# DanielLin94144/E2E-ASR-Pytorch

Measured on NVIDIA B200. Metric: beam-8+LM joint CTC/attn decode utts/sec, higher is better.
Workload: dtype f32

## Files before the change

e2e-asr-pytorch_b200/_lib.py:

```python
import ctypes
import os

from . import build as _build

c_int, c_float, c_void_p = ctypes.c_int, ctypes.c_float, ctypes.c_void_p

CTC_LOGZERO = -100000000.0
DEC_LOG_ZERO = -10000000.0
STATUS_PREFIX_TOO_LONG = 1
STATUS_TOKEN_NOT_CAND = 2
PREFIX_FULL = 1
PREFIX_SKIP_DEAD_ROWS = 2
PREFIX_FAST_MATH = 4
PREFIX_LIBM_MATH = 8
PREFIX_ROW_COPIES = 16
PREFIX_POLY_MATH = 32
PREFIX_POLY_ESTRIN = 64
BEAM_USE_CTC = 1
BEAM_USE_LM = 2

SIGNATURES = {
    "e2e_last_error": (ctypes.c_char_p, []),
    "e2e_abi_version": (c_int, []),
    "e2e_padded_vocab": (c_int, [c_int]),
    "e2e_launch_count": (ctypes.c_longlong, []),
    "e2e_add_launch_count": (None, [ctypes.c_longlong]),
    "e2e_ctc_log_softmax": (c_int, [c_void_p, c_int, c_int, c_int, c_void_p, c_int, c_void_p, c_int, c_void_p]),
    "e2e_ctc_init_state": (c_int, [c_void_p, c_int, c_int, c_int, c_void_p, c_void_p, c_void_p]),
    "e2e_ctc_prefix_score": (c_int, [c_void_p, c_int, c_int, c_int, c_int, c_void_p,
                                     c_void_p, c_int,
                                     c_void_p, c_void_p, c_void_p,
                                     c_void_p, c_void_p, c_int, c_int, c_int,
                                     c_void_p, c_void_p, c_void_p, c_int, c_void_p]),
    "e2e_ctc_prefix_step_supported": (c_int, [c_int, c_int, c_int]),
    "e2e_ctc_prefix_step": (c_int, [c_void_p, c_int, c_int, c_int, c_int, c_void_p,
                                    c_void_p, c_int,
                                    c_void_p, c_void_p, c_void_p, c_void_p,
                                    c_void_p, c_void_p, c_int, c_int, c_int,
                                    c_void_p, c_void_p, c_void_p, c_int, c_void_p]),
    "e2e_beam_candidates": (c_int, [c_void_p, c_int, c_int, c_int, c_int, c_int, c_void_p, c_void_p, c_void_p, c_void_p]),
    "e2e_beam_combine_prune": (c_int, [c_void_p, c_int, c_void_p,
                                       c_void_p, c_int,
                                       c_void_p, c_void_p,
                                       c_int, c_int, c_int, c_int, c_int,
                                       c_void_p, c_void_p,
                                       c_float, c_float, c_float, c_int,
                                       c_void_p, c_void_p, c_void_p, c_void_p,
                                       c_void_p, c_void_p, c_void_p,
                                       c_void_p,
                                       c_void_p, c_void_p, c_void_p,
                                       c_void_p, c_void_p, c_void_p, c_void_p, c_void_p,
                                       c_int, c_void_p, c_int, c_void_p, c_void_p, c_void_p, c_void_p]),
    "e2e_attention_loc_full": (c_int, [c_void_p, c_void_p, c_void_p, c_void_p, c_void_p, c_void_p, c_void_p, c_void_p,
                                       c_float, c_float, c_int, c_int, c_int, c_int, c_int, c_int, c_int, c_int,
                                       c_void_p, c_void_p, c_void_p]),
    "e2e_attention_loc_heads_supported": (c_int, [c_int, c_int, c_int, c_int, c_int]),
    "e2e_attention_loc_heads": (c_int, [c_void_p, c_void_p, c_void_p, c_void_p, c_void_p, c_void_p, c_void_p, c_void_p,
                                        c_float, c_float, c_int, c_int, c_int, c_int, c_int, c_int, c_int, c_int,
                                        c_int, c_int, c_void_p, c_void_p, c_void_p]),
    "e2e_lstm_split_rows": (c_int, [c_void_p, ctypes.c_longlong, c_void_p, c_int, c_int, c_void_p, ctypes.c_longlong, c_int, c_int, c_void_p]),
    "e2e_lstm_split_rows_multi": (c_int, [c_int, c_void_p, c_void_p, c_void_p, c_void_p, c_void_p, c_void_p, c_void_p, c_void_p, c_int, c_void_p]),
    "e2e_lstm_cell": (c_int, [c_void_p, ctypes.c_longlong, c_void_p, c_void_p, c_void_p, c_void_p, c_void_p, c_int, c_int,
                              c_void_p, c_void_p, c_void_p, ctypes.c_longlong, c_int, c_int, c_void_p]),
    "e2e_lstm_split_rows_f16x2": (c_int, [c_void_p, ctypes.c_longlong, c_void_p, c_int, c_int, c_void_p, ctypes.c_longlong, c_int, c_int,
                                          c_float, c_void_p]),
    "e2e_lstm_split_rows_multi_f16x2": (c_int, [c_int, c_void_p, c_void_p, c_void_p, c_void_p, c_void_p, c_void_p, c_void_p, c_void_p,
                                                c_int, c_float, c_void_p]),
    "e2e_lstm_cell_f16x2": (c_int, [c_void_p, ctypes.c_longlong, c_float, c_void_p, c_void_p, c_void_p, c_void_p, c_void_p, c_int, c_int,
                                    c_void_p, c_void_p, c_void_p, ctypes.c_longlong, c_int, c_int, c_float, c_void_p]),
    "e2e_gru_cell": (c_int, [c_void_p, ctypes.c_longlong, c_void_p, c_void_p, c_void_p, c_void_p, c_void_p, c_int, c_int,
                             c_void_p, c_void_p, ctypes.c_longlong, c_int, c_int, c_void_p]),
    "e2e_gru_cell_f16x2": (c_int, [c_void_p, ctypes.c_longlong, c_float, c_void_p, c_void_p, c_void_p, c_void_p, c_void_p, c_int, c_int,
                                   c_void_p, c_void_p, ctypes.c_longlong, c_int, c_int, c_float, c_void_p]),
    "e2e_conv3x3_unfold_split": (c_int, [c_void_p, c_void_p, c_int, c_int, c_int, c_int, ctypes.c_longlong, c_int, c_void_p, c_void_p]),
    "e2e_conv_bias_relu_mask": (c_int, [c_void_p, c_void_p, c_void_p, c_int, c_int, c_int, c_int, ctypes.c_longlong,
                                        ctypes.c_longlong, c_void_p]),
    "e2e_conv3x3_igemm_supported": (c_int, [c_int, c_int]),
    "e2e_conv3x3_igemm": (c_int, [c_void_p, c_void_p, c_int, c_int, c_int, c_int, c_void_p, c_void_p, c_int, c_int, c_void_p, c_void_p]),
    "e2e_lstm_sequence": (c_int, [c_void_p, ctypes.c_longlong, c_void_p, ctypes.c_longlong, c_void_p, c_void_p, c_void_p, c_void_p,
                                  c_int, c_int, c_int, c_int,
                                  c_void_p, c_void_p, c_int, c_int, c_void_p, c_void_p, c_int, c_int, c_void_p]),
    "e2e_gru_sequence": (c_int, [c_void_p, ctypes.c_longlong, c_void_p, ctypes.c_longlong, c_void_p, c_void_p, c_void_p, c_void_p,
                                 c_int, c_int, c_int, c_int,
                                 c_void_p, c_void_p, c_int, c_int, c_void_p, c_void_p, c_int, c_int, c_void_p]),
    "e2e_conv1_direct": (c_int, [c_void_p, ctypes.c_longlong, c_void_p, c_void_p, c_void_p, c_int, c_int, c_int, c_int, c_int,
                                 c_void_p, c_void_p]),
    "e2e_conv_bias_relu_mask_pool": (c_int, [c_void_p, c_void_p, c_void_p, c_int, c_int, c_int, c_int, c_void_p, c_void_p]),
    "e2e_conv1_direct_amax": (c_int, [c_void_p, ctypes.c_longlong, c_void_p, c_void_p, c_void_p, c_int, c_int, c_int, c_int, c_int,
                                      c_void_p, c_void_p, c_void_p]),
    "e2e_conv3x3_unfold_split_f16x2": (c_int, [c_void_p, c_void_p, c_int, c_int, c_int, c_int, ctypes.c_longlong, c_int, c_void_p,
                                               c_void_p, c_void_p]),
    "e2e_conv_bias_relu_mask_scaled": (c_int, [c_void_p, c_void_p, c_void_p, c_int, c_int, c_int, c_int, ctypes.c_longlong,
                                               ctypes.c_longlong, c_void_p, c_float, c_void_p, c_void_p]),
    "e2e_conv_bias_relu_mask_pool_scaled": (c_int, [c_void_p, c_void_p, c_void_p, c_int, c_int, c_int, c_int, c_void_p, c_void_p, c_float,
                                                    c_void_p, c_void_p]),
    "e2e_nbest_pack_ragged": (c_int, [c_int, c_int, c_int, c_void_p, c_void_p, c_void_p, c_void_p, c_void_p, c_void_p, c_void_p,
                                      c_void_p, c_void_p, c_void_p, c_void_p, c_void_p]),
    "e2e_copy_rows_h2d": (c_int, [c_void_p, c_void_p, ctypes.c_longlong, c_int, c_void_p, c_void_p, c_int, c_int, c_void_p, c_void_p]),
    "e2e_beam_finalize": (c_int, [c_int, c_int, c_void_p,
                                  c_void_p, c_void_p,
                                  c_void_p, c_void_p, c_void_p,
                                  c_void_p, c_void_p, c_void_p,
                                  c_void_p, c_void_p, c_int,
                                  c_void_p, c_void_p, c_void_p, c_void_p, c_void_p,
                                  c_int, c_void_p]),
}

_lib = None


class E2EError(RuntimeError):
    pass


def load():
    global _lib
    if _lib is None:
        path = os.environ.get("E2E_ASR_B200_LIB")
        if not path:
            path = _build.LIB_PATH
            if _build.stale():
                path = _build.build()
        lib = ctypes.CDLL(path)
        for name, (res, args) in SIGNATURES.items():
            fn = getattr(lib, name)
            fn.restype, fn.argtypes = res, args
        if lib.e2e_abi_version() != 1:
            raise E2EError("libe2e_asr_b200.so ABI version mismatch")
        _lib = lib
    return _lib


def check(rc):
    if rc != 0:
        raise E2EError("libe2e_asr_b200: rc=%d: %s" % (rc, load().e2e_last_error().decode()))


def ptr(t):
    return None if t is None else t.data_ptr()


def require_cuda(*tensors):
    for t in tensors:
        if t is not None and not t.is_cuda:
            raise E2EError("libe2e_asr_b200 has no CPU path: tensor on %s" % t.device)
```

e2e-asr-pytorch_b200/csrc/conv_igemm.cu:

```cuda
#include "common.cuh"
#include "conv_igemm.cuh"
#include <cuda_bf16.h>

namespace e2e {
namespace {

constexpr int kBM = kIgemmBM, kBN = kIgemmBN, kBK = kIgemmBK;
constexpr int kTile = kBM * kBK * 2;
constexpr int kBStages = 6;
constexpr int kBarBytes = 256;
constexpr int kGroups = 3;
constexpr int kAStages = 2 * kGroups;
constexpr int kThreads = 64 + 128 * kGroups;
constexpr int kSmemBytes = 1024 + (kAStages + kBStages) * kTile + kBarBytes + kBM * 16;

static_assert((2 * (kAStages + kBStages) + 1) * 8 + 4 <= kBarBytes, "barrier block");

constexpr uint32_t kIdesc = (1u << 4) | (1u << 7) | (1u << 10) | ((uint32_t)(kBN >> 3) << 17) | ((uint32_t)(kBM >> 4) << 24);

__device__ __forceinline__ uint64_t sw128_desc(uint32_t saddr)
{
    return (uint64_t)((saddr >> 4) & 0x3fffu) | ((uint64_t)1 << 16) | ((uint64_t)(1024 >> 4) << 32) | ((uint64_t)1 << 46) |
           ((uint64_t)2 << 61);
}

__device__ __forceinline__ void mbar_arrive(uint64_t *bar)
{
    asm volatile("mbarrier.arrive.shared::cta.b64 _, [%0];" ::"r"(smem_u32(bar)) : "memory");
}

__device__ __forceinline__ void tma_load_2d(void *dst, const CUtensorMap *map, int c0, int c1, uint64_t *bar)
{
    asm volatile("cp.async.bulk.tensor.2d.shared::cluster.global.tile.mbarrier::complete_tx::bytes [%0], [%1, {%2, %3}], [%4];"
                 ::"r"(smem_u32(dst)), "l"(map), "r"(c0), "r"(c1), "r"(smem_u32(bar))
                 : "memory");
}

__device__ __forceinline__ void tc_fence_after() { asm volatile("tcgen05.fence::after_thread_sync;" ::: "memory"); }
__device__ __forceinline__ void tc_fence_before() { asm volatile("tcgen05.fence::before_thread_sync;" ::: "memory"); }

__device__ __forceinline__ void tc_mma(uint32_t d_tmem, uint64_t adesc, uint64_t bdesc, uint32_t accumulate)
{
    asm volatile("{\n\t.reg .pred p;\n\tsetp.ne.b32 p, %4, 0;\n\t"
                 "tcgen05.mma.cta_group::1.kind::f16 [%0], %1, %2, %3, p;\n\t}"
                 ::"r"(d_tmem), "l"(adesc), "l"(bdesc), "r"(kIdesc), "r"(accumulate));
}

__device__ __forceinline__ void tc_commit(uint64_t *bar)
{
    asm volatile("tcgen05.commit.cta_group::1.mbarrier::arrive::one.shared::cluster.b64 [%0];" ::"r"(smem_u32(bar)) : "memory");
}

__device__ __forceinline__ void tmem_ld32(uint32_t taddr, float (&v)[32])
{
    uint32_t *r = reinterpret_cast<uint32_t *>(v);
    asm volatile("tcgen05.ld.sync.aligned.32x32b.x32.b32 {%0, %1, %2, %3, %4, %5, %6, %7, %8, %9, %10, %11, %12, %13, %14, %15, "
                 "%16, %17, %18, %19, %20, %21, %22, %23, %24, %25, %26, %27, %28, %29, %30, %31}, [%32];"
                 : "=r"(r[0]), "=r"(r[1]), "=r"(r[2]), "=r"(r[3]), "=r"(r[4]), "=r"(r[5]), "=r"(r[6]), "=r"(r[7]),
                   "=r"(r[8]), "=r"(r[9]), "=r"(r[10]), "=r"(r[11]), "=r"(r[12]), "=r"(r[13]), "=r"(r[14]), "=r"(r[15]),
                   "=r"(r[16]), "=r"(r[17]), "=r"(r[18]), "=r"(r[19]), "=r"(r[20]), "=r"(r[21]), "=r"(r[22]), "=r"(r[23]),
                   "=r"(r[24]), "=r"(r[25]), "=r"(r[26]), "=r"(r[27]), "=r"(r[28]), "=r"(r[29]), "=r"(r[30]), "=r"(r[31])
                 : "r"(taddr));
}

__device__ __forceinline__ uint32_t split_piece2(float x0, float x1, int pp)
{
    __nv_bfloat162 p = __floats2bfloat162_rn(x0, x1);
    if (pp > 0) {
        const float2 a = __bfloat1622float2(p);
        x0 = __fsub_rn(x0, a.x);
        x1 = __fsub_rn(x1, a.y);
        p = __floats2bfloat162_rn(x0, x1);
        if (pp > 1) {
            const float2 b = __bfloat1622float2(p);
            p = __floats2bfloat162_rn(__fsub_rn(x0, b.x), __fsub_rn(x1, b.y));
        }
    }
    return *reinterpret_cast<uint32_t *>(&p);
}

struct alignas(16) IgemmRow {
    const float *pix;
    uint32_t flags;
    uint32_t pad;
};
constexpr uint32_t kRowLive = 1u << 9, kRowPixel = 1u << 10;

__global__ void __launch_bounds__(kThreads, 1)
conv3x3_igemm_kernel(const __grid_constant__ CUtensorMap wmap, const IgemmArgs args)
{
    extern __shared__ uint8_t igemm_smem_raw[];
    uint8_t *smem = reinterpret_cast<uint8_t *>((reinterpret_cast<uintptr_t>(igemm_smem_raw) + 1023) & ~(uintptr_t)1023);
    uint8_t *a_ring = smem;
    uint8_t *b_ring = smem + kAStages * kTile;
    uint64_t *bars = reinterpret_cast<uint64_t *>(b_ring + kBStages * kTile);
    uint64_t *a_full = bars, *a_empty = bars + kAStages;
    uint64_t *b_full = bars + 2 * kAStages, *b_empty = b_full + kBStages;
    uint64_t *acc_full = b_empty + kBStages;
    uint32_t *tmem_slot = reinterpret_cast<uint32_t *>(acc_full + 1);
    IgemmRow *rows = reinterpret_cast<IgemmRow *>(reinterpret_cast<uint8_t *>(bars) + kBarBytes);

    const int warp = threadIdx.x >> 5, lane = threadIdx.x & 31;
    const int H = args.H, W = args.W, C = args.C;
    const bool pool = args.epi == kEpiPool;
    const int n0 = blockIdx.y * kBN;
    const int KB = 9 * C / kBK;

    if (threadIdx.x == 0) {
        for (int i = 0; i < kAStages; ++i) { mbar_init(a_full + i, 128); mbar_init(a_empty + i, 1); }
        for (int i = 0; i < kBStages; ++i) { mbar_init(b_full + i, 1); mbar_init(b_empty + i, 1); }
        mbar_init(acc_full, 1);
        mbar_fence_init();
    }
    if (warp == 0) {
        asm volatile("tcgen05.alloc.cta_group::1.sync.aligned.shared::cta.b32 [%0], 512;" ::"r"(smem_u32(tmem_slot)) : "memory");
        asm volatile("tcgen05.relinquish_alloc_permit.cta_group::1.sync.aligned;" ::: "memory");
    }
    if (threadIdx.x >= 64 && threadIdx.x < 64 + kBM) {
        const int m = threadIdx.x - 64;
        int h = 0, w = 0, n = -1;
        if (pool) {
            const int H2 = (H + 1) >> 1, W2 = (W + 1) >> 1;
            const long long q = (long long)blockIdx.x * (kBM / 4) + (m >> 2);
            if (q < (long long)args.N * H2 * W2) {
                const int w2 = (int)(q % W2);
                const long long t = q / W2;
                h = 2 * (int)(t % H2) + ((m >> 1) & 1);
                w = 2 * w2 + (m & 1);
                if (h < H && w < W) n = (int)(t / H2);
            }
        } else {
            const long long p = (long long)blockIdx.x * kBM + m;
            if (p < (long long)args.N * H * W) {
                const long long t = p / W;
                w = (int)(p % W);
                h = (int)(t % H);
                n = (int)(t / H);
            }
        }
        IgemmRow r = {args.in, 0u, 0u};
        if (n >= 0) {
            const int vr = __ldg(args.valid + n);
            r.pix = args.in + (((long long)n * H + h) * W + w) * C;
            r.flags = kRowPixel | (h < vr ? kRowLive : 0u);
            for (int t = 0; t < 9; ++t) {
                const int hs = h + t / 3 - 1, ws = w + t % 3 - 1;
                if (hs >= 0 && hs < H && hs < vr && ws >= 0 && ws < W) r.flags |= 1u << t;
            }
        }
        rows[m] = r;
    }
    tc_fence_before();
    __syncthreads();
    tc_fence_after();
    const uint32_t tmem = *tmem_slot;

    if (warp == 0) {
        if (lane == 0) {
            int stage = 0;
            uint32_t phase = 0;
            for (int pp = 0; pp < 3; ++pp)
                for (int kb = 0; kb < KB; ++kb)
                    for (int j = 0; j < 3 - pp; ++j) {
                        mbar_wait(b_empty + stage, phase ^ 1u);
                        mbar_arrive_expect_tx(b_full + stage, kTile);
                        tma_load_2d(b_ring + stage * kTile, &wmap, kb * kBK, j * args.Cout + n0, b_full + stage);
                        if (++stage == kBStages) { stage = 0; phase ^= 1u; }
                    }
        }
    } else if (warp == 1) {
        if (lane == 0) {
            int as = 0, bs = 0;
            uint32_t aph = 0, bph = 0;
            for (int pp = 0; pp < 3; ++pp)
                for (int kb = 0; kb < KB; ++kb) {
                    mbar_wait(a_full + as, aph);
                    tc_fence_after();
                    const uint64_t adesc = sw128_desc(smem_u32(a_ring + as * kTile));
                    for (int j = 0; j < 3 - pp; ++j) {
                        mbar_wait(b_full + bs, bph);
                        tc_fence_after();
                        const uint64_t bdesc = sw128_desc(smem_u32(b_ring + bs * kTile));
#pragma unroll
                        for (int k16 = 0; k16 < kBK / 16; ++k16)
                            tc_mma(tmem + (uint32_t)((pp + j) * kBN), adesc + 2 * k16, bdesc + 2 * k16,
                                   (pp > 0 || kb > 0 || k16 > 0) ? 1u : 0u);
                        tc_commit(b_empty + bs);
                        if (++bs == kBStages) { bs = 0; bph ^= 1u; }
                    }
                    tc_commit(a_empty + as);
                    if (++as == kAStages) { as = 0; aph ^= 1u; }
                }
            tc_commit(acc_full);
        }
    } else {
        const int grp = (threadIdx.x - 64) >> 7, pt = (threadIdx.x - 64) & 127;
        const int c16 = pt & 15, rsub = pt >> 4;
        const int cpb = C / kBK;
        int as = grp;
        uint32_t aph = 0;
        for (int seq = grp; seq < 3 * KB; seq += kGroups) {
            const int pp = seq / KB, kb = seq - pp * KB, tap = kb / cpb, cb = kb - tap * cpb;
            const long long tap_off = ((long long)(tap / 3 - 1) * W + (tap % 3 - 1)) * C + cb * kBK + c16 * 4;
            float4 v[kBM / 8];
#pragma unroll
            for (int i = 0; i < kBM / 8; ++i) {
                const IgemmRow r = rows[i * 8 + rsub];
                v[i] = make_float4(0.0f, 0.0f, 0.0f, 0.0f);
                if ((r.flags >> tap) & 1u) v[i] = __ldg(reinterpret_cast<const float4 *>(r.pix + tap_off));
            }
            mbar_wait(a_empty + as, aph ^ 1u);
            uint8_t *tile = a_ring + as * kTile;
#pragma unroll
            for (int i = 0; i < kBM / 8; ++i) {
                const int row = i * 8 + rsub;
                const uint32_t lo = split_piece2(v[i].x, v[i].y, pp), hi = split_piece2(v[i].z, v[i].w, pp);
                const int chunk = (c16 >> 1) ^ (row & 7);
                *reinterpret_cast<uint2 *>(tile + row * 128 + chunk * 16 + (c16 & 1) * 8) = make_uint2(lo, hi);
            }
            asm volatile("fence.proxy.async.shared::cta;" ::: "memory");
            mbar_arrive(a_full + as);
            as += kGroups;
            if (as >= kAStages) { as -= kAStages; aph ^= 1u; }
        }

        const int m = (warp & 3) * 32 + lane;
        const uint32_t flags = rows[m].flags;
        mbar_wait(acc_full, 0);
        tc_fence_after();
        const uint32_t lane_addr = tmem + ((uint32_t)((warp & 3) * 32) << 16);
        const long long H2W2 = (long long)((H + 1) >> 1) * ((W + 1) >> 1);
        const bool live = (flags & kRowLive) != 0u, pixel = (flags & kRowPixel) != 0u;
        for (int c = grp; c < kBN / 32; c += kGroups) {
            float y0[32], y1[32], y2[32];
            tmem_ld32(lane_addr + c * 32, y0);
            tmem_ld32(lane_addr + kBN + c * 32, y1);
            tmem_ld32(lane_addr + 2 * kBN + c * 32, y2);
            asm volatile("tcgen05.wait::ld.sync.aligned;" ::: "memory");
            float y[32];
#pragma unroll
            for (int i = 0; i < 32; ++i) y[i] = __fadd_rn(y0[i], __fadd_rn(y1[i], y2[i]));
            const int col = n0 + c * 32;
            if (args.epi == kEpiRaw) {
                if (pixel) {
                    float4 *dst = reinterpret_cast<float4 *>(args.out + ((long long)blockIdx.x * kBM + m) * args.Cout + col);
#pragma unroll
                    for (int i = 0; i < 8; ++i) dst[i] = make_float4(y[4 * i], y[4 * i + 1], y[4 * i + 2], y[4 * i + 3]);
                }
            } else if (!pool) {
                if (pixel) {
                    float4 *dst = reinterpret_cast<float4 *>(args.out + ((long long)blockIdx.x * kBM + m) * args.Cout + col);
#pragma unroll
                    for (int i = 0; i < 8; ++i) {
                        float4 o = make_float4(0.0f, 0.0f, 0.0f, 0.0f);
                        if (live) {
                            const float4 b = __ldg(reinterpret_cast<const float4 *>(args.bias + col) + i);
                            o.x = fmaxf(__fadd_rn(y[4 * i], b.x), 0.0f); o.y = fmaxf(__fadd_rn(y[4 * i + 1], b.y), 0.0f);
                            o.z = fmaxf(__fadd_rn(y[4 * i + 2], b.z), 0.0f); o.w = fmaxf(__fadd_rn(y[4 * i + 3], b.w), 0.0f);
                        }
                        dst[i] = o;
                    }
                }
            } else {
                const int s = m & 3, base = lane & ~3;
                float t[32];
#pragma unroll
                for (int i = 0; i < 32; ++i) t[i] = live ? __fadd_rn(y[i], __ldg(args.bias + col + i)) : -INFINITY;
                float res[8];
#pragma unroll
                for (int i = 0; i < 32; ++i) {
                    float acc = 0.0f;
#pragma unroll
                    for (int k = 0; k < 4; ++k) acc = fmaxf(acc, __shfl_sync(E2E_FULL_MASK, t[i], base + k));
                    if ((i >> 3) == s) res[i & 7] = acc;
                }
                const long long q = (long long)blockIdx.x * (kBM / 4) + (m >> 2);
                if (q < (long long)args.N * H2W2) {
                    float4 *dst = reinterpret_cast<float4 *>(args.out + q * args.Cout + col + 8 * s);
                    dst[0] = make_float4(res[0], res[1], res[2], res[3]);
                    dst[1] = make_float4(res[4], res[5], res[6], res[7]);
                }
            }
        }
        tc_fence_before();
    }
    __syncthreads();
    if (warp == 0) asm volatile("tcgen05.dealloc.cta_group::1.sync.aligned.b32 %0, 512;" ::"r"(tmem) : "memory");
}

}
}

extern "C" int e2e_tc_conv3x3_igemm_launch(const CUtensorMap *wmap, const e2e::IgemmArgs *args, unsigned tiles, void *stream)
{
    using namespace e2e;
    static bool attr_set = false;
    if (!attr_set) {
        const cudaError_t e = cudaFuncSetAttribute(conv3x3_igemm_kernel, cudaFuncAttributeMaxDynamicSharedMemorySize, kSmemBytes);
        if (e != cudaSuccess) return (int)e;
        attr_set = true;
    }
    conv3x3_igemm_kernel<<<dim3(tiles, (unsigned)(args->Cout / kBN)), kThreads, kSmemBytes, static_cast<cudaStream_t>(stream)>>>(*wmap, *args);
    return (int)cudaGetLastError();
}
```

e2e-asr-pytorch_b200/csrc/conv_igemm.cuh:

```cuda
#pragma once
#include <cuda.h>
#include <cuda_runtime.h>

namespace e2e {

constexpr int kIgemmBM = 128;
constexpr int kIgemmBN = 128;
constexpr int kIgemmBK = 64;

enum { kEpiRaw = 0, kEpiRelu = 1, kEpiPool = 2 };

struct IgemmArgs {
    const float *in;
    const int *valid;
    const float *bias;
    float *out;
    int N, H, W, C, Cout, epi;
};

}

extern "C" int e2e_tc_conv3x3_igemm_launch(const CUtensorMap *wmap, const e2e::IgemmArgs *args, unsigned tiles, void *stream);
```

e2e-asr-pytorch_b200/csrc/conv_igemm_host.cu:

```cuda
#include "common.cuh"
#include "conv_igemm.cuh"

namespace e2e {

typedef CUresult (*EncodeTiledFn)(CUtensorMap *, CUtensorMapDataType, cuuint32_t, void *, const cuuint64_t *, const cuuint64_t *,
                                  const cuuint32_t *, const cuuint32_t *, CUtensorMapInterleave, CUtensorMapSwizzle,
                                  CUtensorMapL2promotion, CUtensorMapFloatOOBfill);
EncodeTiledFn tensor_map_encoder();

namespace {

bool igemm_shape_ok(int C, int Cout)
{
    return (C == 128 || C == 256) && (Cout == 128 || Cout == 256);
}

}
}

using namespace e2e;

extern "C" int e2e_conv3x3_igemm_supported(int C, int Cout)
{
    return igemm_shape_ok(C, Cout) ? 1 : 0;
}

extern "C" int e2e_conv3x3_igemm(const float *in_nhwc, const int *valid_rows, int N, int H, int W, int C,
                                 const void *w_split_bf16, const float *bias, int Cout, int epilogue, float *out, void *stream)
{
    const char *name = "e2e_conv3x3_igemm";
    if (!in_nhwc || !valid_rows || !w_split_bf16 || !out || (epilogue != kEpiRaw && !bias))
        return set_error(E2E_ERR_ARG, "%s: null pointer", name);
    if (N <= 0 || H <= 0 || W <= 0 || epilogue < kEpiRaw || epilogue > kEpiPool)
        return set_error(E2E_ERR_ARG, "%s: bad size or epilogue", name);
    if (!igemm_shape_ok(C, Cout)) return set_error(E2E_ERR_UNSUPPORTED, "%s: C = %d, Cout = %d not supported", name, C, Cout);
    if ((reinterpret_cast<uintptr_t>(in_nhwc) & 15) || (reinterpret_cast<uintptr_t>(w_split_bf16) & 15) ||
        (reinterpret_cast<uintptr_t>(out) & 15) || (reinterpret_cast<uintptr_t>(bias) & 15))
        return set_error(E2E_ERR_ARG, "%s: misaligned buffer", name);
    const long long rows_out = epilogue == kEpiPool ? (long long)N * ((H + 1) / 2) * ((W + 1) / 2) : (long long)N * H * W;
    const long long tiles = epilogue == kEpiPool ? (rows_out + kIgemmBM / 4 - 1) / (kIgemmBM / 4) : (rows_out + kIgemmBM - 1) / kIgemmBM;
    if (tiles > 0x7fffffffLL) return set_error(E2E_ERR_ARG, "%s: too many pixels", name);

    EncodeTiledFn enc = tensor_map_encoder();
    if (!enc) return set_error(E2E_ERR_LAUNCH, "%s: cuTensorMapEncodeTiled is not available from this driver", name);
    CUtensorMap map;
    const cuuint64_t dims[2] = {(cuuint64_t)9 * C, (cuuint64_t)3 * Cout};
    const cuuint64_t strides[1] = {(cuuint64_t)9 * C * 2};
    const cuuint32_t box[2] = {(cuuint32_t)kIgemmBK, (cuuint32_t)kIgemmBN};
    const cuuint32_t estr[2] = {1u, 1u};
    const CUresult cr = enc(&map, CU_TENSOR_MAP_DATA_TYPE_BFLOAT16, 2, const_cast<void *>(w_split_bf16), dims, strides, box, estr,
                            CU_TENSOR_MAP_INTERLEAVE_NONE, CU_TENSOR_MAP_SWIZZLE_128B, CU_TENSOR_MAP_L2_PROMOTION_L2_256B,
                            CU_TENSOR_MAP_FLOAT_OOB_FILL_NONE);
    if (cr != CUDA_SUCCESS) return set_error(E2E_ERR_LAUNCH, "%s: cuTensorMapEncodeTiled failed (CUresult %d)", name, (int)cr);

    const IgemmArgs a = {in_nhwc, valid_rows, bias, out, N, H, W, C, Cout, epilogue};
    const int e = e2e_tc_conv3x3_igemm_launch(&map, &a, (unsigned)tiles, stream);
    count_launch();
    if (e != (int)cudaSuccess) return set_error(E2E_ERR_LAUNCH, "%s: %s", name, cudaGetErrorString((cudaError_t)e));
    return check_launch(name);
}
```

e2e-asr-pytorch_b200/model.py:

```python
import math

import numpy as np
import torch
from torch import nn
import torch.nn.functional as F

FBANK_SIZE = 40


def reference_init_(module):
    if isinstance(module, nn.Embedding):
        module.weight.data.normal_(0, 1)
        return
    for p in module.parameters():
        d = p.data
        if d.dim() == 1:
            d.zero_()
        elif d.dim() == 2:
            d.normal_(0, 1.0 / math.sqrt(d.size(1)))
        elif d.dim() in (3, 4):
            fan = d.size(1)
            for k in d.size()[2:]:
                fan *= k
            d.normal_(0, 1.0 / math.sqrt(fan))
        else:
            raise NotImplementedError


def split_gemm_rows(x, lin, a_bytes=3 << 30):
    from . import ops
    f, k = x.shape
    m_out = lin.b0.shape[1]
    y = torch.empty((f, m_out), dtype=torch.float32, device=x.device)
    blk = max(1, min(f, a_bytes // (3 * k * 2)))
    a = torch.empty((blk, 3 * k), dtype=torch.bfloat16, device=x.device)
    for r0 in range(0, f, blk):
        m = min(blk, f - r0)
        ops.lstm_split_rows(x[r0:r0 + m], None, m, a, k, 0)
        am, ym = a[:m], y[r0:r0 + m]
        torch.mm(am, lin.b2, out_dtype=torch.float32, out=ym)
        torch.addmm(ym, am[:, :2 * k], lin.b1, out_dtype=torch.float32, out=ym)
        torch.addmm(ym, am[:, :k], lin.b0, out_dtype=torch.float32, out=ym)
    return y


class VGGFrontEnd(nn.Module):

    def __init__(self, input_dim):
        super().__init__()
        if input_dim % 13 == 0:
            self.in_channel, self.freq_dim = input_dim // 13, 13
        elif input_dim % FBANK_SIZE == 0:
            self.in_channel, self.freq_dim = input_dim // FBANK_SIZE, FBANK_SIZE
        else:
            raise ValueError("VGG front end needs 13k (MFCC) or 40k (fbank) features, got %d" % input_dim)
        c1, c2 = 128, 256
        self.out_dim = (self.freq_dim // 4) * c2
        self.extractor = nn.Sequential(
            nn.Conv2d(self.in_channel, c1, 3, stride=1, padding=1), nn.ReLU(),
            nn.Conv2d(c1, c1, 3, stride=1, padding=1), nn.ReLU(),
            nn.MaxPool2d(2, stride=2, ceil_mode=True),
            nn.Conv2d(c1, c2, 3, stride=1, padding=1), nn.ReLU(),
            nn.Conv2d(c2, c2, 3, stride=1, padding=1), nn.ReLU(),
            nn.MaxPool2d(2, stride=2, ceil_mode=True))

    def _as_image(self, feat):
        drop = feat.shape[1] % 4
        if drop:
            feat = feat[:, :-drop, :].contiguous()
        n, t, _ = feat.shape
        return feat.view(n, t, self.in_channel, self.freq_dim).transpose(1, 2)

    def forward(self, feat, feat_len):
        img = self.extractor(self._as_image(feat))
        out = img.transpose(1, 2).contiguous()
        return out.view(out.shape[0], out.shape[1], self.out_dim), feat_len // 4

    def forward_masked(self, feat, feat_len):
        img = self._as_image(feat)
        n, _, t, _ = img.shape
        own = (feat_len // 4 * 4).to(img.device)

        def keep(a):
            valid = own // (t // a.shape[2])
            m = torch.arange(a.shape[2], device=a.device)[None, :] < valid[:, None]
            return a * m[:, None, :, None].to(a.dtype)

        img = keep(img)
        for layer in self.extractor:
            img = layer(img)
            if isinstance(layer, nn.ReLU):
                img = keep(img)
        out = img.transpose(1, 2).contiguous()
        return out.view(out.shape[0], out.shape[1], self.out_dim), feat_len // 4


    A_BYTES = 3 << 30

    conv_split_format = "bf16x3"
    conv_path = "igemm"
    IGEMM_MAX_COUT = 128

    def _split_weights(self, conv):
        from .stepper import SplitLinear, SplitLinearF16
        cache = self.__dict__.setdefault("_split_cache", {})
        key = (id(conv), conv.weight.device, self.conv_split_format)
        if key not in cache:
            w2d = conv.weight.detach().permute(2, 3, 1, 0).reshape(-1, conv.out_channels).t().contiguous()
            cache[key] = SplitLinearF16(w2d, act_scale=1.0) if self.conv_split_format == "fp16x2" else SplitLinear(w2d)
        return cache[key]

    def _igemm_weights(self, conv):
        cache = self.__dict__.setdefault("_split_cache", {})
        key = (id(conv), conv.weight.device, "igemm")
        if key not in cache:
            lin, k = self._split_weights(conv), 9 * conv.in_channels
            cache[key] = torch.stack([lin.b0.t(), lin.b1[:k].t(), lin.b2[:k].t()]).contiguous()
        return cache[key]

    def _conv_split(self, x, valid, conv, pool=False, amax_in=None, amax_out=None):
        from . import ops
        n, h, w, c = x.shape
        bias = conv.bias.detach().float().contiguous()
        if (amax_in is None and self.conv_path == "igemm" and conv.out_channels <= self.IGEMM_MAX_COUT
                and ops.conv3x3_igemm_supported(c, conv.out_channels)):
            return ops.conv3x3_igemm(x, valid, self._igemm_weights(conv), bias, "pool" if pool else "relu")
        k = 9 * c
        lin = self._split_weights(conv)
        total = n * h * w
        f16 = amax_in is not None
        pieces, a_dtype = (2, torch.float16) if f16 else (3, torch.bfloat16)
        blk = max(1, min(total, self.A_BYTES // (pieces * k * 2)))
        a = torch.empty((blk, pieces * k), dtype=a_dtype, device=x.device)
        y = torch.empty((total, conv.out_channels), dtype=torch.float32, device=x.device)
        for p0 in range(0, total, blk):
            m = min(blk, total - p0)
            ops.conv3x3_unfold_split(x, valid, p0, m, a, amax=amax_in)
            am, ym = a[:m], y[p0:p0 + m]
            if f16:
                torch.mm(am, lin.b1, out_dtype=torch.float32, out=ym)
            else:
                torch.mm(am, lin.b2, out_dtype=torch.float32, out=ym)
                torch.addmm(ym, am[:, :2 * k], lin.b1, out_dtype=torch.float32, out=ym)
            torch.addmm(ym, am[:, :k], lin.b0, out_dtype=torch.float32, out=ym)
        y = y.view(n, h, w, conv.out_channels)
        scale_args = (amax_in, lin.out_scale, amax_out) if f16 else ()
        if pool:
            return ops.conv_bias_relu_mask_pool(y, bias, valid, *scale_args)
        ops.conv_bias_relu_mask(y, bias, valid, *scale_args)
        return y

    def forward_masked_split(self, feat, feat_len):
        from . import ops
        drop = feat.shape[1] % 4
        if drop:
            feat = feat[:, :-drop, :]
        if feat.stride(2) != 1 or feat.stride(1) != feat.shape[2]:
            feat = feat.contiguous()
        own = (feat_len // 4 * 4).to(feat.device)
        v1 = own.to(torch.int32).contiguous()
        v2 = (own // 2).to(torch.int32).contiguous()
        convs = [m for m in self.extractor if isinstance(m, nn.Conv2d)]
        w1 = convs[0].weight.detach().float().contiguous()
        f16 = self.conv_split_format == "fp16x2"
        amax = torch.zeros(4, dtype=torch.int32, device=feat.device) if f16 else None
        word = lambda i: amax[i:i + 1] if f16 else None
        y = ops.conv1_direct(feat, w1, convs[0].bias.detach().float().contiguous(), v1, self.freq_dim, amax_out=word(0))
        y = self._conv_split(y, v1, convs[1], pool=True, amax_in=word(0), amax_out=word(1))
        y = self._conv_split(y, v2, convs[2], amax_in=word(1), amax_out=word(2))
        y = self._conv_split(y, v2, convs[3], pool=True, amax_in=word(2), amax_out=word(3))
        out = y.permute(0, 1, 3, 2).contiguous()
        return out.view(out.shape[0], out.shape[1], self.out_dim), feat_len // 4


class RecurrentLayer(nn.Module):

    def __init__(self, input_dim, module, dim, bidirection, dropout, layer_norm, sample_rate, sample_style, proj):
        super().__init__()
        if sample_style not in ("drop", "concat"):
            raise ValueError("Unsupported Sample Style: " + sample_style)
        width = 2 * dim if bidirection else dim
        self.out_dim = sample_rate * width if (sample_rate > 1 and sample_style == "concat") else width
        self.sample_rate, self.sample_style = sample_rate, sample_style
        self.dropout, self.layer_norm, self.proj = dropout, layer_norm, proj
        self.layer = getattr(nn, module.upper())(input_dim, dim, bidirectional=bidirection, num_layers=1, batch_first=True)
        if layer_norm:
            self.ln = nn.LayerNorm(width)
        if dropout > 0:
            self.dp = nn.Dropout(p=dropout)
        if proj:
            self.pj = nn.Linear(width, width)

    def _post(self, out, x_len):
        if self.layer_norm:
            out = self.ln(out)
        if self.dropout > 0:
            out = self.dp(out)
        if self.sample_rate > 1:
            n, t, d = out.shape
            x_len = x_len // self.sample_rate
            if self.sample_style == "drop":
                out = out[:, ::self.sample_rate, :].contiguous()
            else:
                if t % self.sample_rate:
                    out = out[:, :-(t % self.sample_rate), :]
                out = out.contiguous().view(n, t // self.sample_rate, d * self.sample_rate)
        if self.proj:
            out = torch.tanh(self.pj(out))
        return out, x_len

    def forward(self, x, x_len):
        out, _ = self.layer(x)
        return self._post(out, x_len)

    def forward_ragged(self, x, x_len):
        rnn = self.layer
        if not rnn.bidirectional:
            out, _ = rnn(x)
            return self._post(out, x_len)
        n, t, _ = x.shape
        fn = torch._VF.lstm if isinstance(rnn, nn.LSTM) else torch._VF.gru
        zeros = x.new_zeros(1, n, rnn.hidden_size)
        hx = (zeros, zeros) if isinstance(rnn, nn.LSTM) else zeros
        names = ("weight_ih_l0", "weight_hh_l0", "bias_ih_l0", "bias_hh_l0")
        w_fw = [getattr(rnn, k) for k in names]
        w_bw = [getattr(rnn, k + "_reverse") for k in names]
        ar = torch.arange(t, device=x.device)[None, :]
        ln = x_len.to(x.device).clamp(min=1)[:, None]
        rev = torch.where(ar < ln, ln - 1 - ar, ar)
        gather = rev[:, :, None]
        fw = fn(x, hx, w_fw, True, 1, 0.0, False, False, True)[0]
        x_rev = x.gather(1, gather.expand(n, t, x.shape[2]))
        bw = fn(x_rev, hx, w_bw, True, 1, 0.0, False, False, True)[0]
        bw = bw.gather(1, gather.expand(n, t, bw.shape[2]))
        return self._post(torch.cat([fw, bw], dim=-1), x_len)


    def packed_supported(self):
        rnn = self.layer
        return (isinstance(rnn, (nn.LSTM, nn.GRU)) and rnn.num_layers == 1 and self.sample_rate == 1 and not self.layer_norm
                and rnn.hidden_size <= 384)

    def _packed_weights(self):
        from .stepper import SplitLinear
        rnn = self.layer
        cache = self.__dict__.setdefault("_packed_cache", {})
        key = rnn.weight_hh_l0.device
        if key not in cache:
            sfx = ["", "_reverse"] if rnn.bidirectional else [""]
            g = lambda n: getattr(rnn, n).detach().float()
            h = rnn.hidden_size
            w_in = torch.cat([g("weight_ih_l0" + x) for x in sfx], dim=0)
            if isinstance(rnn, nn.LSTM):
                dirs = [((g("bias_ih_l0" + x) + g("bias_hh_l0" + x)).contiguous(),
                         g("weight_hh_l0" + x).view(4, h, h).permute(2, 1, 0).contiguous())
                        for x in sfx]
            else:
                dirs = []
                for x in sfx:
                    b_ih, b_hh, w_hh = g("bias_ih_l0" + x), g("bias_hh_l0" + x), g("weight_hh_l0" + x).view(3, h, h)
                    bias = torch.cat([b_ih[:2 * h] + b_hh[:2 * h], b_ih[2 * h:], b_hh[2 * h:]]).contiguous()
                    w_t = torch.cat([w_hh, w_hh.new_zeros(1, h, h)]).permute(2, 1, 0).contiguous()
                    dirs.append((bias, w_t))
            pj = (SplitLinear(self.pj.weight.detach().float()), self.pj.bias.detach().float()) if self.proj else None
            cache[key] = (SplitLinear(w_in), dirs, pj)
        return cache[key]

    def forward_packed(self, x, frame_off, lens32, group_first, group_rows):
        from . import ops
        lin_in, dirs, pj = self._packed_weights()
        h = self.layer.hidden_size
        gru = isinstance(self.layer, nn.GRU)
        n_gates = 3 if gru else 4
        gates = split_gemm_rows(x.contiguous(), lin_in)
        out = torch.empty((x.shape[0], h * len(dirs)), dtype=torch.float32, device=x.device)
        fw = (dirs[0][0], dirs[0][1], 0, 0)
        bw = (dirs[1][0], dirs[1][1], n_gates * h, h) if len(dirs) == 2 else None
        (ops.gru_sequence if gru else ops.lstm_sequence)(gates, out, frame_off, lens32, group_first, group_rows, h, fw, bw)
        if pj is not None:
            out = torch.tanh(split_gemm_rows(out, pj[0]).add_(pj[1]))
        return out


class Encoder(nn.Module):

    def __init__(self, input_size, batch_size, vgg, vgg_freq, vgg_low_filt, module, bidirection, dim, dropout,
                 layer_norm, proj, sample_rate, sample_style):
        super().__init__()
        assert len(sample_rate) == len(dropout) == len(dim), "Number of layer mismatch"
        self.vgg, self.vgg_freq, self.vgg_low_filt = vgg, vgg_freq, vgg_low_filt
        self.sample_rate = 1
        stack, width = [], input_size
        if vgg == 1:
            stack.append(VGGFrontEnd(input_size))
            width = stack[-1].out_dim
            self.sample_rate *= 4
        elif vgg != 0:
            raise NotImplementedError("vgg = {} front end is outside the decode hot path scope".format(vgg))
        if module not in ("LSTM", "GRU"):
            raise NotImplementedError("encoder module " + str(module))
        for l in range(len(dim)):
            stack.append(RecurrentLayer(width, module, dim[l], bidirection, dropout[l], layer_norm[l],
                                        sample_rate[l], sample_style, proj[l]))
            width = stack[-1].out_dim
            self.sample_rate *= sample_rate[l]
        self.in_dim, self.out_dim = input_size, width
        self.layers = nn.ModuleList(stack)

    def forward(self, x, x_len):
        for layer in self.layers:
            x, x_len = layer(x, x_len)
        return x, x_len

    def packed_supported(self):
        return all(isinstance(l, VGGFrontEnd) or (isinstance(l, RecurrentLayer) and l.packed_supported()) for l in self.layers)

    @staticmethod
    def _groups(t_host):
        first, rows, i, n = [], [], 0, len(t_host)
        while i < n:
            t = int(t_host[i])
            r = 4 if t >= 600 else (8 if t >= 300 else 16)
            r = min(r, n - i)
            first.append(i)
            rows.append(r)
            i += r
        return first, rows

    def forward_ragged_packed(self, x, x_len, chunk=128):
        lens_host = x_len.cpu()
        n_utts = x.shape[0]
        front = self.layers[0] if isinstance(self.layers[0], VGGFrontEnd) else None
        packs, tls = [], []
        ready = getattr(self, "chunk_ready", None)
        for lo in range(0, n_utts, chunk):
            hi = min(n_utts, lo + chunk)
            if ready is not None:
                ready(lo, hi)
            l_max = int(lens_host[lo:hi].max())
            xc, lc = x[lo:hi, :l_max], x_len[lo:hi]
            if front is not None:
                if getattr(self, "split_conv", False):
                    xc, lc = front.forward_masked_split(xc, lc)
                else:
                    xc, lc = front.forward_masked(xc, lc)
            lc = lc.to(x.device).reshape(-1)
            mask = torch.arange(xc.shape[1], device=x.device)[None, :] < lc[:, None]
            packs.append(xc[mask])
            tls.append(lc)
        feat = torch.cat(packs, dim=0)
        t_len = torch.cat(tls).long()
        t_host = t_len.cpu()
        frame_off = (torch.cumsum(t_len, 0) - t_len).to(torch.int32).contiguous()
        lens32 = t_len.to(torch.int32).contiguous()
        first, rows = self._groups(t_host)
        g_first = torch.tensor(first, dtype=torch.int32, device=x.device)
        g_rows = torch.tensor(rows, dtype=torch.int32, device=x.device)
        for layer in self.layers:
            if isinstance(layer, RecurrentLayer):
                feat = layer.forward_packed(feat, frame_off, lens32, g_first, g_rows)
        t_max = int(t_host.max())
        enc = feat.new_zeros((n_utts, t_max, feat.shape[1]))
        enc[torch.arange(t_max, device=x.device)[None, :] < t_len[:, None]] = feat
        return enc, t_len

    def forward_ragged(self, x, x_len):
        for layer in self.layers:
            if isinstance(layer, VGGFrontEnd):
                if getattr(self, "split_conv", False) and x.is_cuda:
                    x, x_len = layer.forward_masked_split(x, x_len)
                else:
                    x, x_len = layer.forward_masked(x, x_len)
            else:
                x, x_len = layer.forward_ragged(x, x_len)
        return x, x_len


class _AttentionCore(nn.Module):

    def __init__(self, temperature, num_head):
        super().__init__()
        self.temperature, self.num_head = temperature, num_head
        self.mask, self.k_len = None, None

    def reset_mem(self):
        self.mask, self.k_len = None, None

    def set_mem(self, prev_att):
        pass

    def compute_mask(self, k, k_len):
        self.k_len = k_len
        n, t, _ = k.shape
        pad = torch.arange(t, device=k_len.device)[None, :] >= k_len[:, None]
        self.mask = pad[:, None, :].expand(n, self.num_head, t).reshape(-1, t)

    def _attend(self, energy, value):
        score = (energy / self.temperature).masked_fill(self.mask, -np.inf)
        attn = torch.softmax(score, dim=-1)
        return torch.bmm(attn.unsqueeze(1), value).squeeze(1), attn


class ScaleDotAttention(_AttentionCore):
    def forward(self, q, k, v):
        energy = torch.bmm(q.unsqueeze(1), k.transpose(1, 2)).squeeze(1)
        out, attn = self._attend(energy, v)
        return out, attn.view(-1, self.num_head, k.shape[1])


class LocationAwareAttention(_AttentionCore):

    def __init__(self, kernel_size, kernel_num, dim, num_head, temperature):
        super().__init__(temperature, num_head)
        self.prev_att = None
        self.loc_conv = nn.Conv1d(num_head, kernel_num, kernel_size=2 * kernel_size + 1, padding=kernel_size, bias=False)
        self.loc_proj = nn.Linear(kernel_num, dim, bias=False)
        self.gen_energy = nn.Linear(dim, 1)
        self.dim = dim

    def reset_mem(self):
        super().reset_mem()
        self.prev_att = None

    def set_mem(self, prev_att):
        self.prev_att = prev_att

    def forward(self, q, k, v):
        nh, t, _ = k.shape
        n = nh // self.num_head
        if self.prev_att is None:
            self.prev_att = torch.zeros((n, self.num_head, t), device=k.device)
            for i, sl in enumerate(self.k_len):
                self.prev_att[i, :, :sl] = 1.0 / sl
        loc = torch.tanh(self.loc_proj(self.loc_conv(self.prev_att).transpose(1, 2)))
        loc = loc.unsqueeze(1).repeat(1, self.num_head, 1, 1).view(-1, t, self.dim)
        energy = self.gen_energy(torch.tanh(k + q.unsqueeze(1) + loc)).squeeze(2)
        out, attn = self._attend(energy, v)
        attn = attn.view(n, self.num_head, t)
        self.prev_att = attn
        return out, attn


class Attention(nn.Module):

    def __init__(self, v_dim, q_dim, mode, dim, num_head, temperature, v_proj, loc_kernel_size, loc_kernel_num):
        super().__init__()
        self.v_dim, self.dim, self.mode, self.num_head, self.v_proj = v_dim, dim, mode.lower(), num_head, v_proj
        self.proj_q = nn.Linear(q_dim, dim * num_head)
        self.proj_k = nn.Linear(v_dim, dim * num_head)
        if v_proj:
            self.proj_v = nn.Linear(v_dim, v_dim * num_head)
        if self.mode == "dot":
            self.att_layer = ScaleDotAttention(temperature, num_head)
        elif self.mode == "loc":
            self.att_layer = LocationAwareAttention(loc_kernel_size, loc_kernel_num, dim, num_head, temperature)
        else:
            raise NotImplementedError
        if num_head > 1:
            self.merge_head = nn.Linear(v_dim * num_head, v_dim)
        self.key = self.value = self.mask = None

    def reset_mem(self):
        self.key = self.value = self.mask = None
        self.att_layer.reset_mem()

    def set_mem(self, prev_attn):
        self.att_layer.set_mem(prev_attn)

    def forward(self, dec_state, enc_feat, enc_len):
        n, t, _ = enc_feat.shape
        query = torch.tanh(self.proj_q(dec_state)).view(n * self.num_head, self.dim)
        if self.key is None:
            self.att_layer.compute_mask(enc_feat, enc_len.to(enc_feat.device))
            self.key = torch.tanh(self.proj_k(enc_feat))
            self.value = torch.tanh(self.proj_v(enc_feat)) if self.v_proj else enc_feat
            if self.num_head > 1:
                self.key = self.key.view(n, t, self.num_head, self.dim).permute(0, 2, 1, 3).contiguous().view(-1, t, self.dim)
                if self.v_proj:
                    self.value = self.value.view(n, t, self.num_head, self.v_dim).permute(0, 2, 1, 3).contiguous().view(-1, t, self.v_dim)
                else:
                    self.value = self.value.repeat(self.num_head, 1, 1)
        context, attn = self.att_layer(query, self.key, self.value)
        if self.num_head > 1:
            context = self.merge_head(context.view(n, self.num_head * self.v_dim))
        return attn, context


class Decoder(nn.Module):

    def __init__(self, batch_size, input_dim, vocab_size, module, dim, layer, dropout):
        super().__init__()
        if module not in ("LSTM", "GRU"):
            raise NotImplementedError("decoder module " + str(module))
        self.in_dim, self.layer, self.dim, self.dropout = input_dim, layer, dim, dropout
        self.hidden_state = None
        self.enable_cell = module == "LSTM"
        self.layers = getattr(nn, module)(input_dim, dim, num_layers=layer, dropout=dropout, batch_first=True)
        self.char_trans = nn.Linear(dim, vocab_size)
        self.final_dropout = nn.Dropout(dropout)

    def init_state(self, bs):
        dev = next(self.parameters()).device
        z = lambda: torch.zeros((self.layer, bs, self.dim), device=dev)
        self.hidden_state = (z(), z()) if self.enable_cell else z()
        return self.get_state()

    def set_state(self, hidden_state):
        dev = next(self.parameters()).device
        if self.enable_cell:
            self.hidden_state = (hidden_state[0].to(dev), hidden_state[1].to(dev))
        else:
            self.hidden_state = hidden_state.to(dev)

    def get_state(self):
        if self.enable_cell:
            return (self.hidden_state[0].cpu(), self.hidden_state[1].cpu())
        return self.hidden_state.cpu()

    def get_query(self):
        h = self.hidden_state[0] if self.enable_cell else self.hidden_state
        return h.transpose(0, 1).reshape(-1, self.dim * self.layer)

    def forward(self, x):
        x, self.hidden_state = self.layers(x.unsqueeze(1), self.hidden_state)
        x = x.squeeze(1)
        return self.char_trans(self.final_dropout(x)), x


class ASR(nn.Module):

    def __init__(self, input_size, vocab_size, batch_size, ctc_weight, encoder, attention, decoder,
                 emb_drop=0.0, init_adadelta=True):
        super().__init__()
        assert 0 <= ctc_weight <= 1
        self.vocab_size, self.ctc_weight = vocab_size, ctc_weight
        self.enable_ctc, self.enable_att = ctc_weight > 0, ctc_weight != 1
        self.lm = None
        self.encoder = Encoder(input_size, batch_size, **encoder)
        if self.enable_ctc:
            self.ctc_layer = nn.Sequential(nn.Linear(self.encoder.out_dim, vocab_size), nn.ReLU())
        if self.enable_att:
            self.dec_dim = decoder["dim"]
            self.pre_embed = nn.Embedding(vocab_size, self.dec_dim)
            self.embed_drop = nn.Dropout(emb_drop)
            self.decoder = Decoder(batch_size, self.encoder.out_dim + self.dec_dim, vocab_size, **decoder)
            self.attention = Attention(self.encoder.out_dim, self.dec_dim * self.decoder.layer, **attention)
        self.apply(reference_init_)
        if self.enable_att and self.decoder.enable_cell:
            for l in range(self.decoder.layer):
                b = getattr(self.decoder.layers, "bias_ih_l{}".format(l))
                n = b.size(0)
                b.data[n // 4:n // 2].fill_(1.0)

    def set_state(self, prev_state, prev_attn):
        self.decoder.set_state(prev_state)
        self.attention.set_mem(prev_attn)

    def forward(self, *a, **k):
        raise NotImplementedError("training forward (asr.py:89-177) is outside the decode hot-path scope")


class RNNLM(nn.Module):

    def __init__(self, vocab_size, emb_tying, emb_dim, module, dim, n_layers, dropout):
        super().__init__()
        self.dim, self.n_layers, self.emb_tying, self.vocab_size = dim, n_layers, emb_tying, vocab_size
        if emb_tying:
            assert emb_dim == dim, "Output dim of RNN should be identical to embedding if using weight tying."
        self.emb = nn.Embedding(vocab_size, emb_dim)
        self.dp1, self.dp2 = nn.Dropout(dropout), nn.Dropout(dropout)
        self.rnn = getattr(nn, module.upper())(emb_dim, dim, num_layers=n_layers, dropout=dropout, batch_first=True)
        if not emb_tying:
            self.trans = nn.Linear(emb_dim, vocab_size)

    def forward(self, x, lens, hidden=None):
        emb = self.dp1(self.emb(x))
        packed = nn.utils.rnn.pack_padded_sequence(emb, lens, batch_first=True, enforce_sorted=False)
        out, hidden = self.rnn(packed, hidden)
        out, _ = nn.utils.rnn.pad_packed_sequence(out, batch_first=True)
        out = F.linear(self.dp2(out), self.emb.weight) if self.emb_tying else self.trans(self.dp2(out))
        return out, hidden
```

e2e-asr-pytorch_b200/ops.py:

```python
import torch

from . import _lib as L

I32, F32 = torch.int32, torch.float32


def _stream():
    return torch.cuda.current_stream().cuda_stream


def _chk(t, dtype, name, numel=None):
    if t is None:
        return
    if not t.is_cuda:
        raise L.E2EError("%s must be a CUDA tensor (no CPU path)" % name)
    if t.dtype != dtype:
        raise TypeError("%s must be %s, got %s" % (name, dtype, t.dtype))
    if not t.is_contiguous():
        raise ValueError("%s must be contiguous" % name)
    if numel is not None and t.numel() < numel:
        raise ValueError("%s has %d elements, needs %d" % (name, t.numel(), numel))


def padded_vocab(v):
    return L.load().e2e_padded_vocab(int(v))


def ctc_log_softmax(logits, enc_len=None, apply_relu=True, out=None):
    _chk(logits, F32, "logits")
    _chk(enc_len, I32, "enc_len")
    u, t, v = logits.shape
    vp = padded_vocab(v)
    x = out if out is not None else torch.empty((t, u, vp), dtype=F32, device=logits.device)
    _chk(x, F32, "x", t * u * vp)
    L.check(L.load().e2e_ctc_log_softmax(L.ptr(logits), u, t, v, L.ptr(enc_len), int(bool(apply_relu)),
                                        L.ptr(x), vp, _stream()))
    return x


def ctc_init_state(x, enc_len=None, out=None):
    _chk(x, F32, "x")
    _chk(enc_len, I32, "enc_len")
    t, u, vp = x.shape
    r0 = out if out is not None else torch.empty((u, t, 1, 2), dtype=F32, device=x.device)
    _chk(r0, F32, "r0", u * t * 2)
    L.check(L.load().e2e_ctc_init_state(L.ptr(x), t, u, vp, L.ptr(enc_len), L.ptr(r0), _stream()))
    return r0


def ctc_prefix_score(x, vocab, enc_len, r_prev, prev_lane, last_tok, prefix_len, n_live, cand,
                     beam, n_cand, flags=0, psi=None, r_out=None, status=None, n_run=0):
    t, u, vp = x.shape
    _chk(x, F32, "x")
    _chk(enc_len, I32, "enc_len", u)
    _chk(r_prev, F32, "r_prev")
    lanes_prev = r_prev.shape[2]
    if r_prev.shape[0] != u or r_prev.shape[1] != t or r_prev.shape[3] != 2:
        raise ValueError("r_prev must be [U,Tmax,lanes,2]")
    n = u * beam
    _chk(prev_lane, I32, "prev_lane", n)
    _chk(last_tok, I32, "last_tok", n)
    _chk(prefix_len, I32, "prefix_len", n)
    _chk(n_live, I32, "n_live", u)
    _chk(cand, I32, "cand", n * n_cand)
    if psi is None:
        psi = torch.empty((n, n_cand), dtype=F32, device=x.device)
    if r_out is None:
        r_out = torch.empty((u, t, beam * n_cand, 2), dtype=F32, device=x.device)
    _chk(psi, F32, "psi", n * n_cand)
    _chk(r_out, F32, "r_out", u * t * beam * n_cand * 2)
    _chk(status, I32, "status", u)
    L.check(L.load().e2e_ctc_prefix_score(
        L.ptr(x), t, u, vp, int(vocab), L.ptr(enc_len), L.ptr(r_prev), lanes_prev,
        L.ptr(prev_lane), L.ptr(last_tok), L.ptr(prefix_len), L.ptr(n_live), L.ptr(cand),
        int(beam), int(n_cand), int(flags), L.ptr(psi), L.ptr(r_out), L.ptr(status), int(n_run), _stream()))
    return psi, r_out


def prefix_step_supported(vocab, beam, n_cand):
    return bool(L.load().e2e_ctc_prefix_step_supported(padded_vocab(vocab), int(beam), int(n_cand)))


def ctc_prefix_step(x, vocab, enc_len, r_prev, parent_slot, last_tok, parent_tok, prefix_len, n_live, cand,
                    beam, n_cand, flags=0, psi=None, r_out=None, status=None, n_run=0):
    t, u, vp = x.shape
    _chk(x, F32, "x")
    _chk(enc_len, I32, "enc_len", u)
    _chk(r_prev, F32, "r_prev")
    if r_prev.dim() != 4 or r_prev.shape[0] != u or r_prev.shape[1] != t or r_prev.shape[3] != 2:
        raise ValueError("r_prev must be [U,Tmax,lanes,2]")
    lanes_prev = r_prev.shape[2]
    n = u * beam
    _chk(parent_slot, I32, "parent_slot", n)
    _chk(last_tok, I32, "last_tok", n)
    _chk(parent_tok, I32, "parent_tok", n)
    _chk(prefix_len, I32, "prefix_len", n)
    _chk(n_live, I32, "n_live", u)
    _chk(cand, I32, "cand", n * n_cand)
    if psi is None:
        psi = torch.empty((n, n_cand), dtype=F32, device=x.device)
    if r_out is None:
        r_out = torch.empty((u, t, beam, 2), dtype=F32, device=x.device)
    _chk(psi, F32, "psi", n * n_cand)
    _chk(r_out, F32, "r_out", u * t * beam * 2)
    _chk(status, I32, "status", u)
    L.check(L.load().e2e_ctc_prefix_step(
        L.ptr(x), t, u, vp, int(vocab), L.ptr(enc_len), L.ptr(r_prev), lanes_prev,
        L.ptr(parent_slot), L.ptr(last_tok), L.ptr(parent_tok), L.ptr(prefix_len), L.ptr(n_live), L.ptr(cand),
        int(beam), int(n_cand), int(flags), L.ptr(psi), L.ptr(r_out), L.ptr(status), int(n_run), _stream()))
    return psi, r_out


def beam_candidates(att_logits, n_utts, beam, vocab, n_cand, n_live, att_stats, cand):
    _chk(att_logits, F32, "att_logits")
    ld = att_logits.stride(0) if att_logits.dim() == 2 else vocab
    _chk(n_live, I32, "n_live", n_utts)
    _chk(att_stats, F32, "att_stats", n_utts * beam * 2)
    _chk(cand, I32, "cand", n_utts * beam * n_cand)
    L.check(L.load().e2e_beam_candidates(L.ptr(att_logits), int(ld), int(n_utts), int(beam), int(vocab), int(n_cand),
                                        L.ptr(n_live), L.ptr(att_stats), L.ptr(cand), _stream()))


class BeamBuffers:

    def __init__(self, n_utts, beam, n_cand, max_steps, min_len, max_len, device, fin_cap=None):
        u, b = n_utts, beam
        self.U, self.B, self.C, self.S = u, b, n_cand, max(1, int(max_steps))
        z = lambda *s, dt=I32: torch.zeros(s, dtype=dt, device=device)
        self.min_len = min_len.to(device=device, dtype=I32).contiguous()
        self.max_len = max_len.to(device=device, dtype=I32).contiguous()
        self.n_live = (self.max_len > 0).to(I32)
        self.n_active = self.n_live.clone()
        self.last_tok, self.prefix_len, self.prev_lane = z(u, b), z(u, b), z(u, b)
        self.score_sum, self.ctc_prob = z(u, b, dt=F32), z(u, b, dt=F32)
        self.parent_slot = z(u, b)
        self.parent_row = torch.arange(u * b, dtype=torch.int64, device=device).view(u, b)
        self.last_tok64 = z(u, b, dt=torch.int64)
        self.parent_tok = torch.full((u, b), -1, dtype=I32, device=device)
        self.hist_tok, self.hist_parent = z(self.S, u, b), z(self.S, u, b)
        self.hist_score = z(self.S, u, b, dt=F32)
        self.fin_cap = int(fin_cap if fin_cap is not None else b)
        self.fin_count = z(u)
        self.fin_step, self.fin_parent = z(u, self.fin_cap), z(u, self.fin_cap)
        self.fin_sum, self.fin_score = z(u, self.fin_cap, dt=F32), z(u, self.fin_cap, dt=F32)
        self.status = z(u)
        self.att_stats = z(u * b, 2, dt=F32)
        self.cand = z(u * b, max(1, n_cand))
        self.psi = z(u * b, max(1, n_cand), dt=F32)


def beam_combine_prune(buf, att_logits, lm_logits, vocab, step, ctc_weight, lm_weight, eos_threshold=1.5, n_run=0):
    _chk(att_logits, F32, "att_logits")
    _chk(lm_logits, F32, "lm_logits")
    flags = (L.BEAM_USE_CTC if ctc_weight > 0 else 0) | (L.BEAM_USE_LM if lm_logits is not None else 0)
    L.check(L.load().e2e_beam_combine_prune(
        L.ptr(att_logits), int(att_logits.stride(0)), L.ptr(buf.att_stats),
        L.ptr(lm_logits), int(lm_logits.stride(0)) if lm_logits is not None else 0,
        L.ptr(buf.cand), L.ptr(buf.psi),
        buf.U, buf.B, int(vocab), buf.C, int(step),
        L.ptr(buf.min_len), L.ptr(buf.max_len),
        float(ctc_weight), float(lm_weight), float(eos_threshold), flags,
        L.ptr(buf.n_live), L.ptr(buf.n_active), L.ptr(buf.last_tok), L.ptr(buf.prefix_len),
        L.ptr(buf.score_sum), L.ptr(buf.ctc_prob), L.ptr(buf.prev_lane),
        L.ptr(buf.parent_slot),
        L.ptr(buf.hist_tok), L.ptr(buf.hist_parent), L.ptr(buf.hist_score),
        L.ptr(buf.fin_count), L.ptr(buf.fin_step), L.ptr(buf.fin_parent), L.ptr(buf.fin_sum), L.ptr(buf.fin_score),
        buf.fin_cap, L.ptr(buf.status), int(n_run), L.ptr(buf.parent_row), L.ptr(buf.last_tok64), L.ptr(buf.parent_tok), _stream()))


def beam_finalize(buf, out_cap=None):
    dev = buf.n_live.device
    cap = int(out_cap if out_cap is not None else buf.S + 1)
    tok = torch.zeros((buf.U, buf.B, cap), dtype=I32, device=dev)
    sc = torch.zeros((buf.U, buf.B, cap), dtype=F32, device=dev)
    ln = torch.zeros((buf.U, buf.B), dtype=I32, device=dev)
    avg = torch.zeros((buf.U, buf.B), dtype=F32, device=dev)
    n = torch.zeros((buf.U,), dtype=I32, device=dev)
    L.check(L.load().e2e_beam_finalize(
        buf.U, buf.B, L.ptr(buf.max_len), L.ptr(buf.n_live), L.ptr(buf.score_sum),
        L.ptr(buf.hist_tok), L.ptr(buf.hist_parent), L.ptr(buf.hist_score),
        L.ptr(buf.fin_count), L.ptr(buf.fin_step), L.ptr(buf.fin_parent), L.ptr(buf.fin_sum), L.ptr(buf.fin_score),
        buf.fin_cap, L.ptr(tok), L.ptr(sc), L.ptr(ln), L.ptr(avg), L.ptr(n), cap, _stream()))
    return tok, sc, ln, avg, n


def nbest_pack_ragged(tok, sc, ln, avg, n, slot, tok_off, cap, hdr, tok_out, sc_out):
    u, beam, cap_in = tok.shape
    _chk(tok, I32, "tok"); _chk(sc, F32, "sc"); _chk(ln, I32, "ln", u * beam); _chk(avg, F32, "avg", u * beam); _chk(n, I32, "n", u)
    _chk(slot, I32, "slot", u); _chk(tok_off, torch.int64, "tok_off", u); _chk(cap, I32, "cap", u)
    _chk(hdr, I32, "hdr"); _chk(tok_out, I32, "tok_out"); _chk(sc_out, I32, "sc_out")
    if u == 0:
        return
    L.check(L.load().e2e_nbest_pack_ragged(u, beam, cap_in, L.ptr(tok), L.ptr(sc), L.ptr(ln), L.ptr(avg), L.ptr(n), L.ptr(slot),
                                          L.ptr(tok_off), L.ptr(cap), L.ptr(hdr), L.ptr(tok_out), L.ptr(sc_out), _stream()))


def attention_loc_full(key_t, value, query, prev_att, enc_len, w_conv, w_proj, w_energy, b_energy, temperature, beam,
                       n_run=None, hyps_per_unit=0, attn=None, ctx=None):
    for t, nm in ((key_t, "key_t"), (value, "value"), (query, "query"), (prev_att, "prev_att"), (w_conv, "w_conv"),
                  (w_proj, "w_proj"), (w_energy, "w_energy")):
        _chk(t, F32, nm)
    _chk(enc_len, I32, "enc_len")
    u, a, t_len = key_t.shape
    e = value.shape[2]
    k, w = w_conv.shape
    n_run = u if n_run is None else int(n_run)
    n = n_run * beam
    if value.shape[0] != u or value.shape[1] != t_len or prev_att.shape[1] != t_len or n_run > u:
        raise ValueError("attention_loc_full: inconsistent shapes")
    _chk(query, F32, "query", n * a)
    _chk(prev_att, F32, "prev_att", n * t_len)
    if attn is None:
        attn = torch.empty((n, t_len), dtype=F32, device=key_t.device)
    if ctx is None:
        ctx = torch.empty((n, e), dtype=F32, device=key_t.device)
    _chk(attn, F32, "attn", n * t_len)
    _chk(ctx, F32, "ctx", n * e)
    L.check(L.load().e2e_attention_loc_full(L.ptr(key_t), L.ptr(value), L.ptr(query), L.ptr(prev_att), L.ptr(enc_len),
                                           L.ptr(w_conv), L.ptr(w_proj), L.ptr(w_energy), float(b_energy), float(temperature),
                                           n_run, int(beam), int(t_len), int(a), int(k), int(w), int(e), int(hyps_per_unit),
                                           L.ptr(attn), L.ptr(ctx), _stream()))
    return attn, ctx


def attention_loc_heads_supported(beam, heads, dim, n_filt, width):
    return bool(L.load().e2e_attention_loc_heads_supported(int(beam), int(heads), int(dim), int(n_filt), int(width)))


def attention_loc_heads(key_t, value, query, prev_att, enc_len, w_conv, w_proj, w_energy, b_energy, temperature, beam,
                        per_head_values, n_run=None, hyps_per_unit=0, attn=None, ctx=None):
    for t, nm in ((key_t, "key_t"), (value, "value"), (query, "query"), (prev_att, "prev_att"), (w_conv, "w_conv"),
                  (w_proj, "w_proj"), (w_energy, "w_energy")):
        _chk(t, F32, nm)
    _chk(enc_len, I32, "enc_len")
    u, h, a, t_len = key_t.shape
    k, h_w, w = w_conv.shape
    e = value.shape[2] // h if per_head_values else value.shape[2]
    n_run = u if n_run is None else int(n_run)
    n = n_run * beam
    if (h_w != h or value.shape[0] != u or value.shape[1] != t_len or (per_head_values and value.shape[2] != h * e)
            or prev_att.shape[-1] != t_len or n_run > u):
        raise ValueError("attention_loc_heads: inconsistent shapes")
    _chk(query, F32, "query", n * h * a)
    _chk(prev_att, F32, "prev_att", n * h * t_len)
    if attn is None:
        attn = torch.empty((n, h, t_len), dtype=F32, device=key_t.device)
    if ctx is None:
        ctx = torch.empty((n, h * e), dtype=F32, device=key_t.device)
    _chk(attn, F32, "attn", n * h * t_len)
    _chk(ctx, F32, "ctx", n * h * e)
    L.check(L.load().e2e_attention_loc_heads(L.ptr(key_t), L.ptr(value), L.ptr(query), L.ptr(prev_att), L.ptr(enc_len),
                                            L.ptr(w_conv), L.ptr(w_proj), L.ptr(w_energy), float(b_energy), float(temperature),
                                            n_run, int(beam), int(h), int(t_len), int(a), int(k), int(w), int(e),
                                            int(bool(per_head_values)), int(hyps_per_unit), L.ptr(attn), L.ptr(ctx), _stream()))
    return attn, ctx


def lstm_split_rows(src, row_idx, n, dst, k, off, scale=None):
    pieces = _pieces(dst, scale)
    _chk(src, F32, "src")
    _chk(row_idx, torch.int64, "row_idx", n)
    w = src.shape[1]
    if dst.shape[0] < n or dst.shape[1] < pieces * k:
        raise ValueError("lstm_split_rows: dst too small")
    if row_idx is None and src.shape[0] < n:
        raise ValueError("lstm_split_rows: src has fewer than n rows")
    if pieces == 3:
        L.check(L.load().e2e_lstm_split_rows(L.ptr(src), int(src.stride(0)), L.ptr(row_idx), int(n), int(w),
                                            L.ptr(dst), int(dst.stride(0)), int(k), int(off), _stream()))
    else:
        L.check(L.load().e2e_lstm_split_rows_f16x2(L.ptr(src), int(src.stride(0)), L.ptr(row_idx), int(n), int(w),
                                                  L.ptr(dst), int(dst.stride(0)), int(k), int(off), float(scale), _stream()))


def _pieces(dst, scale):
    if dst is None:
        return 3 if scale is None else 2
    if not dst.is_cuda:
        raise L.E2EError("split operand must be a CUDA tensor (no CPU path)")
    if not dst.is_contiguous():
        raise ValueError("split operand must be contiguous")
    if dst.dtype == torch.bfloat16 and scale is None:
        return 3
    if dst.dtype == torch.float16 and scale is not None:
        return 2
    raise TypeError("split operand must be bf16 (3 pieces, no scale) or fp16 (2 pieces, with a scale), got %s" % dst.dtype)


class SplitPlan:

    def __init__(self, pairs, scale=None):
        import ctypes
        n = len(pairs)
        for src, dst, k, off in pairs:
            _chk(src, F32, "src")
            if _pieces(dst, scale) != (3 if scale is None else 2):
                raise TypeError("SplitPlan: mixed operand formats")
        self.scale = scale
        self.keep = pairs
        self.n = n
        self.srcs = (ctypes.c_void_p * n)(*[p[0].data_ptr() for p in pairs])
        self.src_pitch = (ctypes.c_longlong * n)(*[int(p[0].stride(0)) for p in pairs])
        self.widths = (ctypes.c_int * n)(*[int(p[0].shape[1]) for p in pairs])
        self.dsts = (ctypes.c_void_p * n)(*[p[1].data_ptr() for p in pairs])
        self.dst_pitch = (ctypes.c_longlong * n)(*[int(p[1].stride(0)) for p in pairs])
        self.ks = (ctypes.c_int * n)(*[int(p[2]) for p in pairs])
        self.offs = (ctypes.c_int * n)(*[int(p[3]) for p in pairs])
        self.rows = min(min(p[0].shape[0], p[1].shape[0]) for p in pairs)

    def run(self, row_idx, n_rows):
        if n_rows > self.rows or (row_idx is not None and (row_idx.dtype != torch.int64 or not row_idx.is_cuda or row_idx.numel() < n_rows)):
            raise ValueError("SplitPlan.run: bad row index / row count")
        if self.scale is None:
            L.check(L.load().e2e_lstm_split_rows_multi(self.n, self.srcs, self.src_pitch, self.widths, self.dsts, self.dst_pitch,
                                                      self.ks, self.offs, L.ptr(row_idx), int(n_rows), _stream()))
        else:
            L.check(L.load().e2e_lstm_split_rows_multi_f16x2(self.n, self.srcs, self.src_pitch, self.widths, self.dsts, self.dst_pitch,
                                                            self.ks, self.offs, L.ptr(row_idx), int(n_rows), float(self.scale), _stream()))


def lstm_cell(gates, bias, c_prev, row_idx, n, c_new, h_new, table=None, tok=None, a_next=None, k_next=0, off_next=0,
              gate_scale=None, next_scale=None):
    _chk(gates, F32, "gates")
    _chk(bias, F32, "bias")
    _chk(c_prev, F32, "c_prev")
    _chk(row_idx, torch.int64, "row_idx", n)
    _chk(c_new, F32, "c_new")
    _chk(h_new, F32, "h_new")
    _chk(table, F32, "table")
    _chk(tok, torch.int64, "tok", n)
    f16 = gate_scale is not None
    if a_next is not None and _pieces(a_next, next_scale if f16 else None) != (2 if f16 else 3):
        raise TypeError("lstm_cell: a_next does not match the operand format")
    d = c_prev.shape[1]
    if gates.shape[0] < n or gates.shape[1] < 4 * d or c_new.shape[0] < n or h_new.shape[0] < n or bias.numel() < 4 * d:
        raise ValueError("lstm_cell: inconsistent shapes")
    a_pitch = int(a_next.stride(0)) if a_next is not None else 0
    if not f16:
        L.check(L.load().e2e_lstm_cell(L.ptr(gates), int(gates.stride(0)), L.ptr(bias), L.ptr(table), L.ptr(tok), L.ptr(c_prev),
                                      L.ptr(row_idx), int(n), int(d), L.ptr(c_new), L.ptr(h_new), L.ptr(a_next),
                                      a_pitch, int(k_next), int(off_next), _stream()))
    else:
        L.check(L.load().e2e_lstm_cell_f16x2(L.ptr(gates), int(gates.stride(0)), float(gate_scale), L.ptr(bias), L.ptr(table), L.ptr(tok),
                                            L.ptr(c_prev), L.ptr(row_idx), int(n), int(d), L.ptr(c_new), L.ptr(h_new), L.ptr(a_next),
                                            a_pitch, int(k_next), int(off_next), float(next_scale if next_scale is not None else 1.0),
                                            _stream()))


def gru_cell(gates, bias, h_prev, row_idx, n, h_new, table=None, tok=None, a_next=None, k_next=0, off_next=0,
             gate_scale=None, next_scale=None):
    _chk(gates, F32, "gates")
    _chk(bias, F32, "bias")
    _chk(h_prev, F32, "h_prev")
    _chk(row_idx, torch.int64, "row_idx", n)
    _chk(h_new, F32, "h_new")
    _chk(table, F32, "table")
    _chk(tok, torch.int64, "tok", n)
    f16 = gate_scale is not None
    if a_next is not None and _pieces(a_next, next_scale if f16 else None) != (2 if f16 else 3):
        raise TypeError("gru_cell: a_next does not match the operand format")
    d = h_prev.shape[1]
    if gates.shape[0] < n or gates.shape[1] < 4 * d or h_new.shape[0] < n or bias.numel() < 4 * d:
        raise ValueError("gru_cell: inconsistent shapes")
    if h_new.data_ptr() == h_prev.data_ptr():
        raise ValueError("gru_cell: h_new must not alias h_prev")
    a_pitch = int(a_next.stride(0)) if a_next is not None else 0
    if not f16:
        L.check(L.load().e2e_gru_cell(L.ptr(gates), int(gates.stride(0)), L.ptr(bias), L.ptr(table), L.ptr(tok), L.ptr(h_prev),
                                     L.ptr(row_idx), int(n), int(d), L.ptr(h_new), L.ptr(a_next),
                                     a_pitch, int(k_next), int(off_next), _stream()))
    else:
        L.check(L.load().e2e_gru_cell_f16x2(L.ptr(gates), int(gates.stride(0)), float(gate_scale), L.ptr(bias), L.ptr(table), L.ptr(tok),
                                           L.ptr(h_prev), L.ptr(row_idx), int(n), int(d), L.ptr(h_new), L.ptr(a_next),
                                           a_pitch, int(k_next), int(off_next), float(next_scale if next_scale is not None else 1.0),
                                           _stream()))


def conv3x3_unfold_split(x_nhwc, valid_rows, first_pixel, n_pixels, out, amax=None):
    _chk(x_nhwc, F32, "x_nhwc")
    _chk(valid_rows, I32, "valid_rows", x_nhwc.shape[0])
    n, h, w, c = x_nhwc.shape
    if amax is None:
        _chk(out, torch.bfloat16, "out", n_pixels * 27 * c)
        L.check(L.load().e2e_conv3x3_unfold_split(L.ptr(x_nhwc), L.ptr(valid_rows), n, h, w, c, int(first_pixel), int(n_pixels),
                                                 L.ptr(out), _stream()))
    else:
        _chk(out, torch.float16, "out", n_pixels * 18 * c)
        _chk(amax, I32, "amax", 1)
        L.check(L.load().e2e_conv3x3_unfold_split_f16x2(L.ptr(x_nhwc), L.ptr(valid_rows), n, h, w, c, int(first_pixel), int(n_pixels),
                                                       L.ptr(amax), L.ptr(out), _stream()))


def conv3x3_igemm_supported(c_in, c_out):
    return bool(L.load().e2e_conv3x3_igemm_supported(int(c_in), int(c_out)))


IGEMM_EPILOGUE = {"raw": 0, "relu": 1, "pool": 2}


def conv3x3_igemm(x_nhwc, valid_rows, w_split, bias, epilogue="relu"):
    _chk(x_nhwc, F32, "x_nhwc")
    _chk(valid_rows, I32, "valid_rows", x_nhwc.shape[0])
    _chk(w_split, torch.bfloat16, "w_split")
    n, h, w, c = x_nhwc.shape
    if w_split.dim() != 3 or w_split.shape[0] != 3 or w_split.shape[2] != 9 * c:
        raise ValueError("w_split must be [3, Cout, 9*%d], got %s" % (c, tuple(w_split.shape)))
    cout = w_split.shape[1]
    if epilogue not in IGEMM_EPILOGUE:
        raise ValueError("unknown epilogue " + str(epilogue))
    if epilogue != "raw":
        _chk(bias, F32, "bias", cout)
    if epilogue == "raw":
        out = torch.empty((n * h * w, cout), dtype=F32, device=x_nhwc.device)
    elif epilogue == "relu":
        out = torch.empty((n, h, w, cout), dtype=F32, device=x_nhwc.device)
    else:
        out = torch.empty((n, (h + 1) // 2, (w + 1) // 2, cout), dtype=F32, device=x_nhwc.device)
    L.check(L.load().e2e_conv3x3_igemm(L.ptr(x_nhwc), L.ptr(valid_rows), n, h, w, c, L.ptr(w_split),
                                      L.ptr(bias) if epilogue != "raw" else None, int(cout), IGEMM_EPILOGUE[epilogue],
                                      L.ptr(out), _stream()))
    return out


def conv_bias_relu_mask(y_nhwc, bias, valid_rows, amax_in=None, inv_w_scale=None, amax_out=None):
    _chk(y_nhwc, F32, "y_nhwc")
    _chk(bias, F32, "bias", y_nhwc.shape[3])
    _chk(valid_rows, I32, "valid_rows", y_nhwc.shape[0])
    n, h, w, c = y_nhwc.shape
    if amax_in is None:
        L.check(L.load().e2e_conv_bias_relu_mask(L.ptr(y_nhwc), L.ptr(bias), L.ptr(valid_rows), n, h, w, c, 0, n * h * w, _stream()))
    else:
        _chk(amax_in, I32, "amax_in", 1)
        _chk(amax_out, I32, "amax_out", 1)
        L.check(L.load().e2e_conv_bias_relu_mask_scaled(L.ptr(y_nhwc), L.ptr(bias), L.ptr(valid_rows), n, h, w, c, 0, n * h * w,
                                                       L.ptr(amax_in), float(inv_w_scale), L.ptr(amax_out), _stream()))


def lstm_sequence(gates, out, frame_off, lens, group_first, group_rows, hidden, fw, bw=None):
    _chk(gates, F32, "gates")
    _chk(out, F32, "out")
    for t, nm in ((frame_off, "frame_off"), (lens, "lens"), (group_first, "group_first"), (group_rows, "group_rows")):
        _chk(t, I32, nm)
    dirs = [fw] + ([bw] if bw is not None else [])
    for b, w, _, _ in dirs:
        _chk(b, F32, "bias", 4 * hidden)
        _chk(w, F32, "w_t", 4 * hidden * hidden)
    if bw is None:
        bw = (None, None, 0, 0)
    L.check(L.load().e2e_lstm_sequence(L.ptr(gates), int(gates.stride(0)), L.ptr(out), int(out.stride(0)),
                                      L.ptr(frame_off), L.ptr(lens), L.ptr(group_first), L.ptr(group_rows),
                                      int(lens.numel()), int(hidden), int(group_first.numel()), len(dirs),
                                      L.ptr(fw[0]), L.ptr(fw[1]), int(fw[2]), int(fw[3]),
                                      L.ptr(bw[0]), L.ptr(bw[1]), int(bw[2]), int(bw[3]), _stream()))


def gru_sequence(gates, out, frame_off, lens, group_first, group_rows, hidden, fw, bw=None):
    _chk(gates, F32, "gates")
    _chk(out, F32, "out")
    for t, nm in ((frame_off, "frame_off"), (lens, "lens"), (group_first, "group_first"), (group_rows, "group_rows")):
        _chk(t, I32, nm)
    dirs = [fw] + ([bw] if bw is not None else [])
    for b, w, _, _ in dirs:
        _chk(b, F32, "bias", 4 * hidden)
        _chk(w, F32, "w_t", 4 * hidden * hidden)
    if bw is None:
        bw = (None, None, 0, 0)
    L.check(L.load().e2e_gru_sequence(L.ptr(gates), int(gates.stride(0)), L.ptr(out), int(out.stride(0)),
                                     L.ptr(frame_off), L.ptr(lens), L.ptr(group_first), L.ptr(group_rows),
                                     int(lens.numel()), int(hidden), int(group_first.numel()), len(dirs),
                                     L.ptr(fw[0]), L.ptr(fw[1]), int(fw[2]), int(fw[3]),
                                     L.ptr(bw[0]), L.ptr(bw[1]), int(bw[2]), int(bw[3]), _stream()))


def conv1_direct(feat, weight, bias, valid_rows, n_freq, amax_out=None):
    _chk(weight, F32, "weight")
    _chk(bias, F32, "bias")
    _chk(valid_rows, I32, "valid_rows", feat.shape[0])
    _chk(amax_out, I32, "amax_out", 1)
    if not feat.is_cuda or feat.dtype != F32 or feat.stride(2) != 1 or feat.stride(1) != feat.shape[2]:
        raise ValueError("conv1_direct: feat must be a CUDA fp32 [N,L,D] tensor with contiguous utterances")
    n, l, d = feat.shape
    cout, cin = weight.shape[0], weight.shape[1]
    if d != cin * n_freq:
        raise ValueError("conv1_direct: feature width %d != Cin*F" % d)
    out = torch.empty((n, l, n_freq, cout), dtype=F32, device=feat.device)
    if amax_out is None:
        L.check(L.load().e2e_conv1_direct(L.ptr(feat), int(feat.stride(0)), L.ptr(weight), L.ptr(bias), L.ptr(valid_rows),
                                         n, l, int(n_freq), int(cin), int(cout), L.ptr(out), _stream()))
    else:
        L.check(L.load().e2e_conv1_direct_amax(L.ptr(feat), int(feat.stride(0)), L.ptr(weight), L.ptr(bias), L.ptr(valid_rows),
                                              n, l, int(n_freq), int(cin), int(cout), L.ptr(out), L.ptr(amax_out), _stream()))
    return out


def conv_bias_relu_mask_pool(y_nhwc, bias, valid_rows, amax_in=None, inv_w_scale=None, amax_out=None):
    _chk(y_nhwc, F32, "y_nhwc")
    _chk(bias, F32, "bias", y_nhwc.shape[3])
    _chk(valid_rows, I32, "valid_rows", y_nhwc.shape[0])
    n, h, w, c = y_nhwc.shape
    out = torch.empty((n, (h + 1) // 2, (w + 1) // 2, c), dtype=F32, device=y_nhwc.device)
    if amax_in is None:
        L.check(L.load().e2e_conv_bias_relu_mask_pool(L.ptr(y_nhwc), L.ptr(bias), L.ptr(valid_rows), n, h, w, c, L.ptr(out), _stream()))
    else:
        _chk(amax_in, I32, "amax_in", 1)
        _chk(amax_out, I32, "amax_out", 1)
        L.check(L.load().e2e_conv_bias_relu_mask_pool_scaled(L.ptr(y_nhwc), L.ptr(bias), L.ptr(valid_rows), n, h, w, c, L.ptr(out),
                                                            L.ptr(amax_in), float(inv_w_scale), L.ptr(amax_out), _stream()))
    return out


def launch_count():
    return int(L.load().e2e_launch_count())


def add_launch_count(n):
    L.load().e2e_add_launch_count(int(n))
```

include/e2e_asr_b200.h:

```cpp
#ifndef E2E_ASR_B200_H
#define E2E_ASR_B200_H

#ifdef __cplusplus
extern "C" {
#endif

#define E2E_ABI_VERSION 1

#define E2E_CTC_LOGZERO   (-100000000.0f)
#define E2E_CTC_BLANK     0
#define E2E_CTC_EOS       1
#define E2E_DEC_LOG_ZERO  (-10000000.0f)

#define E2E_OK              0
#define E2E_ERR_ARG        (-1)
#define E2E_ERR_LAUNCH     (-2)
#define E2E_ERR_UNSUPPORTED (-3)

#define E2E_STATUS_PREFIX_TOO_LONG   1
#define E2E_STATUS_TOKEN_NOT_CAND    2

#define E2E_PREFIX_FULL           1
#define E2E_PREFIX_SKIP_DEAD_ROWS 2
#define E2E_PREFIX_FAST_MATH      4
#define E2E_PREFIX_LIBM_MATH      8
#define E2E_PREFIX_ROW_COPIES    16
#define E2E_PREFIX_POLY_MATH     32
#define E2E_PREFIX_POLY_ESTRIN   64

#define E2E_BEAM_USE_CTC 1
#define E2E_BEAM_USE_LM  2

const char *e2e_last_error(void);
int e2e_abi_version(void);
int e2e_padded_vocab(int V);

int e2e_ctc_log_softmax(const float *logits, int U, int Tmax, int V, const int *enc_len,
                        int apply_relu, float *x, int Vp, void *stream);

int e2e_ctc_init_state(const float *x, int Tmax, int U, int Vp, const int *enc_len,
                       float *r0, void *stream);

int e2e_ctc_prefix_score(const float *x, int Tmax, int U, int Vp, int V, const int *enc_len,
                         const float *r_prev, int lanes_prev,
                         const int *prev_lane, const int *last_tok, const int *prefix_len,
                         const int *n_live, const int *cand, int B, int C, int flags,
                         float *psi, float *r_out, int *status, int n_run, void *stream);

int e2e_ctc_prefix_step_supported(int Vp, int B, int C);
int e2e_ctc_prefix_step(const float *x, int Tmax, int U, int Vp, int V, const int *enc_len,
                        const float *r_prev, int lanes_prev,
                        const int *parent_slot, const int *last_tok, const int *parent_tok, const int *prefix_len,
                        const int *n_live, const int *cand, int B, int C, int flags,
                        float *psi, float *r_out, int *status, int n_run, void *stream);

int e2e_beam_candidates(const float *att_logits, int ld, int U, int B, int V, int C,
                        const int *n_live, float *att_stats, int *cand, void *stream);

int e2e_beam_combine_prune(const float *att_logits, int ld_att, const float *att_stats,
                           const float *lm_logits, int ld_lm,
                           const int *cand, const float *psi,
                           int U, int B, int V, int C, int step,
                           const int *min_len, const int *max_len,
                           float ctc_weight, float lm_weight, float eos_threshold, int flags,
                           int *n_live, int *n_active, int *last_tok, int *prefix_len,
                           float *score_sum, float *ctc_prob, int *prev_lane,
                           int *parent_slot,
                           int *hist_tok, int *hist_parent, float *hist_score,
                           int *fin_count, int *fin_step, int *fin_parent, float *fin_sum, float *fin_score,
                           int fin_cap, int *status, int n_run,
                           long long *parent_row, long long *last_tok64, int *parent_tok, void *stream);

int e2e_beam_finalize(int U, int B, const int *max_len,
                      const int *n_live, const float *score_sum,
                      const int *hist_tok, const int *hist_parent, const float *hist_score,
                      const int *fin_count, const int *fin_step, const int *fin_parent,
                      const float *fin_sum, const float *fin_score, int fin_cap,
                      int *out_tok, float *out_score, int *out_len, float *out_avg, int *out_n,
                      int out_cap, void *stream);

int e2e_nbest_pack_ragged(int U, int B, int cap_in, const int *tok, const float *score, const int *len,
                          const float *avg, const int *n, const int *slot, const long long *tok_off,
                          const int *cap, int *hdr, int *tok_out, int *sc_out, void *stream);

int e2e_attention_loc_full(const float *key_t, const float *value, const float *query, const float *prev_att,
                           const int *enc_len, const float *w_conv, const float *w_proj, const float *w_energy,
                           float b_energy, float temperature, int n_run, int B, int T, int A, int K, int W, int E,
                           int hyps_per_unit, float *attn, float *ctx, void *stream);

int e2e_attention_loc_heads_supported(int B, int H, int A, int K, int W);
int e2e_attention_loc_heads(const float *key_t, const float *value, const float *query, const float *prev_att,
                            const int *enc_len, const float *w_conv, const float *w_proj, const float *w_energy,
                            float b_energy, float temperature, int n_run, int B, int H, int T, int A, int K, int W, int E,
                            int per_head_values, int hyps_per_unit, float *attn, float *ctx, void *stream);

int e2e_lstm_split_rows(const float *src, long long src_pitch, const long long *row_idx, int n, int w,
                        void *dst_bf16, long long dst_pitch, int K, int off, void *stream);

int e2e_lstm_split_rows_multi(int n_src, const float *const *srcs_host, const long long *src_pitches_host, const int *widths_host,
                              void *const *dsts_bf16_host, const long long *dst_pitches_host, const int *Ks_host, const int *offs_host,
                              const long long *row_idx, int n, void *stream);

int e2e_lstm_cell(const float *gates, long long gates_pitch, const float *bias, const float *table, const long long *tok,
                  const float *c_prev, const long long *row_idx, int n, int D,
                  float *c_new, float *h_new, void *a_next_bf16, long long a_pitch, int K_next, int off_next,
                  void *stream);

int e2e_lstm_split_rows_f16x2(const float *src, long long src_pitch, const long long *row_idx, int n, int w,
                              void *dst_f16, long long dst_pitch, int K, int off, float scale, void *stream);
int e2e_lstm_split_rows_multi_f16x2(int n_src, const float *const *srcs_host, const long long *src_pitches_host, const int *widths_host,
                                    void *const *dsts_f16_host, const long long *dst_pitches_host, const int *Ks_host, const int *offs_host,
                                    const long long *row_idx, int n, float scale, void *stream);
int e2e_lstm_cell_f16x2(const float *gates, long long gates_pitch, float gate_scale, const float *bias, const float *table,
                        const long long *tok, const float *c_prev, const long long *row_idx, int n, int D,
                        float *c_new, float *h_new, void *a_next_f16, long long a_pitch, int K_next, int off_next,
                        float next_scale, void *stream);

int e2e_gru_cell(const float *gates, long long gates_pitch, const float *bias, const float *table, const long long *tok,
                 const float *h_prev, const long long *row_idx, int n, int D,
                 float *h_new, void *a_next_bf16, long long a_pitch, int K_next, int off_next, void *stream);
int e2e_gru_cell_f16x2(const float *gates, long long gates_pitch, float gate_scale, const float *bias, const float *table,
                       const long long *tok, const float *h_prev, const long long *row_idx, int n, int D,
                       float *h_new, void *a_next_f16, long long a_pitch, int K_next, int off_next, float next_scale, void *stream);

int e2e_conv3x3_unfold_split(const float *in_nhwc, const int *valid_rows, int N, int H, int W, int C,
                             long long first_pixel, int n_pixels, void *out_bf16, void *stream);

int e2e_conv_bias_relu_mask(float *y_nhwc, const float *bias, const int *valid_rows, int N, int H, int W, int C,
                            long long first_pixel, long long n_pixels, void *stream);

int e2e_conv3x3_igemm_supported(int C, int Cout);
int e2e_conv3x3_igemm(const float *in_nhwc, const int *valid_rows, int N, int H, int W, int C,
                      const void *w_split_bf16, const float *bias, int Cout, int epilogue, float *out, void *stream);

int e2e_lstm_sequence(const float *gates, long long gates_pitch, float *out, long long out_pitch,
                      const int *frame_off, const int *lens, const int *group_first, const int *group_rows,
                      int N, int H, int n_groups, int n_dirs,
                      const float *bias_fw, const float *w_t_fw, int gate_off_fw, int out_off_fw,
                      const float *bias_bw, const float *w_t_bw, int gate_off_bw, int out_off_bw,
                      void *stream);

int e2e_gru_sequence(const float *gates, long long gates_pitch, float *out, long long out_pitch,
                     const int *frame_off, const int *lens, const int *group_first, const int *group_rows,
                     int N, int H, int n_groups, int n_dirs,
                     const float *bias_fw, const float *w_t_fw, int gate_off_fw, int out_off_fw,
                     const float *bias_bw, const float *w_t_bw, int gate_off_bw, int out_off_bw,
                     void *stream);

int e2e_conv1_direct(const float *feat, long long feat_pitch_n, const float *weight, const float *bias,
                     const int *valid_rows, int N, int L, int F, int Cin, int Cout, float *out_nhwc, void *stream);

int e2e_conv_bias_relu_mask_pool(const float *y_nhwc, const float *bias, const int *valid_rows, int N, int H, int W, int C,
                                 float *out_nhwc, void *stream);

int e2e_conv1_direct_amax(const float *feat, long long feat_pitch_n, const float *weight, const float *bias,
                          const int *valid_rows, int N, int L, int F, int Cin, int Cout, float *out_nhwc,
                          unsigned *amax_out, void *stream);
int e2e_conv3x3_unfold_split_f16x2(const float *in_nhwc, const int *valid_rows, int N, int H, int W, int C,
                                   long long first_pixel, int n_pixels, const unsigned *amax_in, void *out_f16, void *stream);
int e2e_conv_bias_relu_mask_scaled(float *y_nhwc, const float *bias, const int *valid_rows, int N, int H, int W, int C,
                                   long long first_pixel, long long n_pixels, const unsigned *amax_in, float inv_w_scale,
                                   unsigned *amax_out, void *stream);
int e2e_conv_bias_relu_mask_pool_scaled(const float *y_nhwc, const float *bias, const int *valid_rows, int N, int H, int W, int C,
                                        float *out_nhwc, const unsigned *amax_in, float inv_w_scale, unsigned *amax_out,
                                        void *stream);

int e2e_copy_rows_h2d(const float *host, float *dev, long long row_pitch, int D, const int *lens_host,
                      const long long *order_host, int n, int chunk, void *const *events, void *stream);

long long e2e_launch_count(void);
void e2e_add_launch_count(long long n);

#ifdef __cplusplus
}
#endif
#endif
```

Baseline: 1029.

## Chain VGG conv3x3 igemm layers through pre-split bf16x3 plane buffers

Input activations are now pre-split once into three bf16 planes with a zero sentinel row. The igemm A-producer loads these with cp.async instead of loading fp32 and splitting every tap in registers. The epilogue can write split planes directly, so conv2 to conv3 to conv4 chain without fp32 round trips. All three 3x3 convs, including the 256-channel ones, now take the igemm path, and the grid is flattened to one dimension. The cost is an extra split kernel, a larger bf16 workspace (3x planes), and a per-call cudaMallocAsync in the fp32 entry.

```diff
diff --git a/e2e-asr-pytorch_b200/_lib.py b/e2e-asr-pytorch_b200/_lib.py
--- a/e2e-asr-pytorch_b200/_lib.py
+++ b/e2e-asr-pytorch_b200/_lib.py
@@ -76,6 +76,9 @@
     "e2e_conv_bias_relu_mask": (c_int, [c_void_p, c_void_p, c_void_p, c_int, c_int, c_int, c_int, ctypes.c_longlong,
                                         ctypes.c_longlong, c_void_p]),
     "e2e_conv3x3_igemm_supported": (c_int, [c_int, c_int]),
+    "e2e_conv3x3_split_planes": (c_int, [c_void_p, c_int, c_int, c_int, c_int, c_void_p, c_void_p]),
+    "e2e_conv3x3_igemm_planes": (c_int, [c_void_p, c_void_p, c_int, c_int, c_int, c_int, c_void_p, c_void_p, c_int, c_int, c_int,
+                                         c_void_p, c_void_p]),
     "e2e_conv3x3_igemm": (c_int, [c_void_p, c_void_p, c_int, c_int, c_int, c_int, c_void_p, c_void_p, c_int, c_int, c_void_p, c_void_p]),
     "e2e_lstm_sequence": (c_int, [c_void_p, ctypes.c_longlong, c_void_p, ctypes.c_longlong, c_void_p, c_void_p, c_void_p, c_void_p,
                                   c_int, c_int, c_int, c_int,
diff --git a/e2e-asr-pytorch_b200/csrc/conv_igemm.cu b/e2e-asr-pytorch_b200/csrc/conv_igemm.cu
--- a/e2e-asr-pytorch_b200/csrc/conv_igemm.cu
+++ b/e2e-asr-pytorch_b200/csrc/conv_igemm.cu
@@ -1,6 +1,7 @@
 #include "common.cuh"
 #include "conv_igemm.cuh"
 #include <cuda_bf16.h>
+#include <algorithm>
 
 namespace e2e {
 namespace {
@@ -12,7 +13,7 @@
 constexpr int kGroups = 3;
 constexpr int kAStages = 2 * kGroups;
 constexpr int kThreads = 64 + 128 * kGroups;
-constexpr int kSmemBytes = 1024 + (kAStages + kBStages) * kTile + kBarBytes + kBM * 16;
+constexpr int kSmemBytes = 1024 + (kAStages + kBStages) * kTile + kBarBytes + kBM * 8;
 
 static_assert((2 * (kAStages + kBStages) + 1) * 8 + 4 <= kBarBytes, "barrier block");
 
@@ -22,11 +23,6 @@
 {
     return (uint64_t)((saddr >> 4) & 0x3fffu) | ((uint64_t)1 << 16) | ((uint64_t)(1024 >> 4) << 32) | ((uint64_t)1 << 46) |
            ((uint64_t)2 << 61);
-}
-
-__device__ __forceinline__ void mbar_arrive(uint64_t *bar)
-{
-    asm volatile("mbarrier.arrive.shared::cta.b64 _, [%0];" ::"r"(smem_u32(bar)) : "memory");
 }
 
 __device__ __forceinline__ void tma_load_2d(void *dst, const CUtensorMap *map, int c0, int c1, uint64_t *bar)
@@ -63,26 +59,45 @@
                  : "r"(taddr));
 }
 
-__device__ __forceinline__ uint32_t split_piece2(float x0, float x1, int pp)
-{
-    __nv_bfloat162 p = __floats2bfloat162_rn(x0, x1);
-    if (pp > 0) {
-        const float2 a = __bfloat1622float2(p);
-        x0 = __fsub_rn(x0, a.x);
-        x1 = __fsub_rn(x1, a.y);
-        p = __floats2bfloat162_rn(x0, x1);
-        if (pp > 1) {
-            const float2 b = __bfloat1622float2(p);
-            p = __floats2bfloat162_rn(__fsub_rn(x0, b.x), __fsub_rn(x1, b.y));
-        }
-    }
-    return *reinterpret_cast<uint32_t *>(&p);
-}
-
-struct alignas(16) IgemmRow {
-    const float *pix;
+__device__ __forceinline__ void mbar_arrive(uint64_t *bar)
+{
+    asm volatile("mbarrier.arrive.shared::cta.b64 _, [%0];" ::"r"(smem_u32(bar)) : "memory");
+}
+
+__device__ __forceinline__ void split3(float x0, float x1, uint32_t &p0, uint32_t &p1, uint32_t &p2)
+{
+    const __nv_bfloat162 a = __floats2bfloat162_rn(x0, x1);
+    const float2 af = __bfloat1622float2(a);
+    x0 = __fsub_rn(x0, af.x);
+    x1 = __fsub_rn(x1, af.y);
+    const __nv_bfloat162 b = __floats2bfloat162_rn(x0, x1);
+    const float2 bf = __bfloat1622float2(b);
+    const __nv_bfloat162 c = __floats2bfloat162_rn(__fsub_rn(x0, bf.x), __fsub_rn(x1, bf.y));
+    p0 = *reinterpret_cast<const uint32_t *>(&a);
+    p1 = *reinterpret_cast<const uint32_t *>(&b);
+    p2 = *reinterpret_cast<const uint32_t *>(&c);
+}
+
+__device__ __forceinline__ void store8(const IgemmArgs &a, long long row, int col, const float *v)
+{
+    if (a.out_planes) {
+        uint32_t p[3][4];
+#pragma unroll
+        for (int i = 0; i < 4; ++i) split3(v[2 * i], v[2 * i + 1], p[0][i], p[1][i], p[2][i]);
+        __nv_bfloat16 *dst = static_cast<__nv_bfloat16 *>(a.out) + row * a.Cout + col;
+        const long long plane = (a.rows_out + 1) * a.Cout;
+#pragma unroll
+        for (int pp = 0; pp < 3; ++pp) *reinterpret_cast<uint4 *>(dst + pp * plane) = make_uint4(p[pp][0], p[pp][1], p[pp][2], p[pp][3]);
+    } else {
+        float4 *dst = reinterpret_cast<float4 *>(static_cast<float *>(a.out) + row * a.Cout + col);
+        dst[0] = make_float4(v[0], v[1], v[2], v[3]);
+        dst[1] = make_float4(v[4], v[5], v[6], v[7]);
+    }
+}
+
+struct IgemmRow {
+    int pix;
     uint32_t flags;
-    uint32_t pad;
 };
 constexpr uint32_t kRowLive = 1u << 9, kRowPixel = 1u << 10;
 
@@ -102,8 +117,11 @@
 
     const int warp = threadIdx.x >> 5, lane = threadIdx.x & 31;
     const int H = args.H, W = args.W, C = args.C;
+    const int P = args.N * H * W;
     const bool pool = args.epi == kEpiPool;
-    const int n0 = blockIdx.y * kBN;
+    const int nblk = args.Cout / kBN;
+    const long long tile = blockIdx.x / nblk;
+    const int n0 = (int)(blockIdx.x % nblk) * kBN;
     const int KB = 9 * C / kBK;
 
     if (threadIdx.x == 0) {
@@ -121,8 +139,8 @@
         int h = 0, w = 0, n = -1;
         if (pool) {
             const int H2 = (H + 1) >> 1, W2 = (W + 1) >> 1;
-            const long long q = (long long)blockIdx.x * (kBM / 4) + (m >> 2);
-            if (q < (long long)args.N * H2 * W2) {
+            const long long q = tile * (kBM / 4) + (m >> 2);
+            if (q < args.rows_out) {
                 const int w2 = (int)(q % W2);
                 const long long t = q / W2;
                 h = 2 * (int)(t % H2) + ((m >> 1) & 1);
@@ -130,18 +148,18 @@
                 if (h < H && w < W) n = (int)(t / H2);
             }
         } else {
-            const long long p = (long long)blockIdx.x * kBM + m;
-            if (p < (long long)args.N * H * W) {
+            const long long p = tile * kBM + m;
+            if (p < P) {
                 const long long t = p / W;
                 w = (int)(p % W);
                 h = (int)(t % H);
                 n = (int)(t / H);
             }
         }
-        IgemmRow r = {args.in, 0u, 0u};
+        IgemmRow r = {P, 0u};
         if (n >= 0) {
             const int vr = __ldg(args.valid + n);
-            r.pix = args.in + (((long long)n * H + h) * W + w) * C;
+            r.pix = (n * H + h) * W + w;
             r.flags = kRowPixel | (h < vr ? kRowLive : 0u);
             for (int t = 0; t < 9; ++t) {
                 const int hs = h + t / 3 - 1, ws = w + t % 3 - 1;
@@ -195,41 +213,44 @@
         }
     } else {
         const int grp = (threadIdx.x - 64) >> 7, pt = (threadIdx.x - 64) & 127;
-        const int c16 = pt & 15, rsub = pt >> 4;
+        const int c8 = pt & 7, rsub = pt >> 3;
         const int cpb = C / kBK;
-        int as = grp;
+        const __nv_bfloat16 *planes = static_cast<const __nv_bfloat16 *>(args.in) + c8 * 8;
+        int as = grp, prev = -1;
         uint32_t aph = 0;
         for (int seq = grp; seq < 3 * KB; seq += kGroups) {
             const int pp = seq / KB, kb = seq - pp * KB, tap = kb / cpb, cb = kb - tap * cpb;
-            const long long tap_off = ((long long)(tap / 3 - 1) * W + (tap % 3 - 1)) * C + cb * kBK + c16 * 4;
-            float4 v[kBM / 8];
-#pragma unroll
-            for (int i = 0; i < kBM / 8; ++i) {
-                const IgemmRow r = rows[i * 8 + rsub];
-                v[i] = make_float4(0.0f, 0.0f, 0.0f, 0.0f);
-                if ((r.flags >> tap) & 1u) v[i] = __ldg(reinterpret_cast<const float4 *>(r.pix + tap_off));
-            }
+            const int off = (tap / 3 - 1) * W + (tap % 3 - 1);
+            const __nv_bfloat16 *src = planes + (long long)pp * (P + 1) * C + cb * kBK;
             mbar_wait(a_empty + as, aph ^ 1u);
-            uint8_t *tile = a_ring + as * kTile;
-#pragma unroll
-            for (int i = 0; i < kBM / 8; ++i) {
-                const int row = i * 8 + rsub;
-                const uint32_t lo = split_piece2(v[i].x, v[i].y, pp), hi = split_piece2(v[i].z, v[i].w, pp);
-                const int chunk = (c16 >> 1) ^ (row & 7);
-                *reinterpret_cast<uint2 *>(tile + row * 128 + chunk * 16 + (c16 & 1) * 8) = make_uint2(lo, hi);
-            }
-            asm volatile("fence.proxy.async.shared::cta;" ::: "memory");
-            mbar_arrive(a_full + as);
+            const uint32_t tile = smem_u32(a_ring + as * kTile);
+#pragma unroll
+            for (int i = 0; i < kBM / 16; ++i) {
+                const int row = i * 16 + rsub;
+                const IgemmRow r = rows[row];
+                const int pix = ((r.flags >> tap) & 1u) ? r.pix + off : P;
+                const uint32_t dst = tile + row * 128 + ((c8 ^ (row & 7)) << 4);
+                asm volatile("cp.async.cg.shared.global [%0], [%1], 16;" ::"r"(dst), "l"(src + (long long)pix * C) : "memory");
+            }
+            asm volatile("cp.async.commit_group;" ::: "memory");
+            if (prev >= 0) {
+                asm volatile("cp.async.wait_group 1;" ::: "memory");
+                asm volatile("fence.proxy.async.shared::cta;" ::: "memory");
+                mbar_arrive(a_full + prev);
+            }
+            prev = as;
             as += kGroups;
             if (as >= kAStages) { as -= kAStages; aph ^= 1u; }
         }
+        asm volatile("cp.async.wait_group 0;" ::: "memory");
+        asm volatile("fence.proxy.async.shared::cta;" ::: "memory");
+        mbar_arrive(a_full + prev);
 
         const int m = (warp & 3) * 32 + lane;
         const uint32_t flags = rows[m].flags;
         mbar_wait(acc_full, 0);
         tc_fence_after();
         const uint32_t lane_addr = tmem + ((uint32_t)((warp & 3) * 32) << 16);
-        const long long H2W2 = (long long)((H + 1) >> 1) * ((W + 1) >> 1);
         const bool live = (flags & kRowLive) != 0u, pixel = (flags & kRowPixel) != 0u;
         for (int c = grp; c < kBN / 32; c += kGroups) {
             float y0[32], y1[32], y2[32];
@@ -241,25 +262,15 @@
 #pragma unroll
             for (int i = 0; i < 32; ++i) y[i] = __fadd_rn(y0[i], __fadd_rn(y1[i], y2[i]));
             const int col = n0 + c * 32;
-            if (args.epi == kEpiRaw) {
+            if (!pool) {
                 if (pixel) {
-                    float4 *dst = reinterpret_cast<float4 *>(args.out + ((long long)blockIdx.x * kBM + m) * args.Cout + col);
-#pragma unroll
-                    for (int i = 0; i < 8; ++i) dst[i] = make_float4(y[4 * i], y[4 * i + 1], y[4 * i + 2], y[4 * i + 3]);
-                }
-            } else if (!pool) {
-                if (pixel) {
-                    float4 *dst = reinterpret_cast<float4 *>(args.out + ((long long)blockIdx.x * kBM + m) * args.Cout + col);
-#pragma unroll
-                    for (int i = 0; i < 8; ++i) {
-                        float4 o = make_float4(0.0f, 0.0f, 0.0f, 0.0f);
-                        if (live) {
-                            const float4 b = __ldg(reinterpret_cast<const float4 *>(args.bias + col) + i);
-                            o.x = fmaxf(__fadd_rn(y[4 * i], b.x), 0.0f); o.y = fmaxf(__fadd_rn(y[4 * i + 1], b.y), 0.0f);
-                            o.z = fmaxf(__fadd_rn(y[4 * i + 2], b.z), 0.0f); o.w = fmaxf(__fadd_rn(y[4 * i + 3], b.w), 0.0f);
-                        }
-                        dst[i] = o;
+                    if (args.epi == kEpiRelu) {
+#pragma unroll
+                        for (int i = 0; i < 32; ++i)
+                            y[i] = live ? fmaxf(__fadd_rn(y[i], __ldg(args.bias + col + i)), 0.0f) : 0.0f;
                     }
+#pragma unroll
+                    for (int i = 0; i < 4; ++i) store8(args, tile * kBM + m, col + 8 * i, y + 8 * i);
                 }
             } else {
                 const int s = m & 3, base = lane & ~3;
@@ -274,18 +285,38 @@
                     for (int k = 0; k < 4; ++k) acc = fmaxf(acc, __shfl_sync(E2E_FULL_MASK, t[i], base + k));
                     if ((i >> 3) == s) res[i & 7] = acc;
                 }
-                const long long q = (long long)blockIdx.x * (kBM / 4) + (m >> 2);
-                if (q < (long long)args.N * H2W2) {
-                    float4 *dst = reinterpret_cast<float4 *>(args.out + q * args.Cout + col + 8 * s);
-                    dst[0] = make_float4(res[0], res[1], res[2], res[3]);
-                    dst[1] = make_float4(res[4], res[5], res[6], res[7]);
-                }
-            }
+                const long long q = tile * (kBM / 4) + (m >> 2);
+                if (q < args.rows_out) store8(args, q, col + 8 * s, res);
+            }
+        }
+        if (args.out_planes && blockIdx.x == 0) {
+            __nv_bfloat16 *zero = static_cast<__nv_bfloat16 *>(args.out) + args.rows_out * args.Cout;
+            for (int i = threadIdx.x - 64; i < 3 * args.Cout / 8; i += 128 * kGroups)
+                *reinterpret_cast<uint4 *>(zero + (i / (args.Cout / 8)) * (args.rows_out + 1) * args.Cout + (i % (args.Cout / 8)) * 8) =
+                    make_uint4(0u, 0u, 0u, 0u);
         }
         tc_fence_before();
     }
     __syncthreads();
     if (warp == 0) asm volatile("tcgen05.dealloc.cta_group::1.sync.aligned.b32 %0, 512;" ::"r"(tmem) : "memory");
+}
+
+__global__ void conv3x3_split_kernel(const float *__restrict__ in, long long P, int C, __nv_bfloat16 *__restrict__ planes)
+{
+    const long long groups = (P + 1) * C / 8, plane = (P + 1) * C;
+    for (long long g = blockIdx.x * (long long)blockDim.x + threadIdx.x; g < groups; g += (long long)gridDim.x * blockDim.x) {
+        float v[8] = {0.0f, 0.0f, 0.0f, 0.0f, 0.0f, 0.0f, 0.0f, 0.0f};
+        if (g < P * C / 8) {
+            const float4 a = __ldg(reinterpret_cast<const float4 *>(in) + 2 * g), b = __ldg(reinterpret_cast<const float4 *>(in) + 2 * g + 1);
+            v[0] = a.x; v[1] = a.y; v[2] = a.z; v[3] = a.w; v[4] = b.x; v[5] = b.y; v[6] = b.z; v[7] = b.w;
+        }
+        uint32_t p[3][4];
+#pragma unroll
+        for (int i = 0; i < 4; ++i) split3(v[2 * i], v[2 * i + 1], p[0][i], p[1][i], p[2][i]);
+#pragma unroll
+        for (int pp = 0; pp < 3; ++pp)
+            *reinterpret_cast<uint4 *>(planes + pp * plane + g * 8) = make_uint4(p[pp][0], p[pp][1], p[pp][2], p[pp][3]);
+    }
 }
 
 }
@@ -300,6 +331,15 @@
         if (e != cudaSuccess) return (int)e;
         attr_set = true;
     }
-    conv3x3_igemm_kernel<<<dim3(tiles, (unsigned)(args->Cout / kBN)), kThreads, kSmemBytes, static_cast<cudaStream_t>(stream)>>>(*wmap, *args);
+    conv3x3_igemm_kernel<<<tiles * (unsigned)(args->Cout / kBN), kThreads, kSmemBytes, static_cast<cudaStream_t>(stream)>>>(*wmap, *args);
     return (int)cudaGetLastError();
 }
+
+extern "C" int e2e_tc_conv3x3_split_launch(const float *in, long long P, int C, void *planes, void *stream)
+{
+    using namespace e2e;
+    const long long groups = (P + 1) * C / 8;
+    const unsigned blocks = (unsigned)std::min<long long>((groups + 255) / 256, 148LL * 16);
+    conv3x3_split_kernel<<<blocks, 256, 0, static_cast<cudaStream_t>(stream)>>>(in, P, C, static_cast<__nv_bfloat16 *>(planes));
+    return (int)cudaGetLastError();
+}
diff --git a/e2e-asr-pytorch_b200/csrc/conv_igemm.cuh b/e2e-asr-pytorch_b200/csrc/conv_igemm.cuh
--- a/e2e-asr-pytorch_b200/csrc/conv_igemm.cuh
+++ b/e2e-asr-pytorch_b200/csrc/conv_igemm.cuh
@@ -11,13 +11,16 @@
 enum { kEpiRaw = 0, kEpiRelu = 1, kEpiPool = 2 };
 
 struct IgemmArgs {
-    const float *in;
+    const void *in;
     const int *valid;
     const float *bias;
-    float *out;
+    void *out;
+    long long rows_out;
     int N, H, W, C, Cout, epi;
+    int out_planes;
 };
 
 }
 
 extern "C" int e2e_tc_conv3x3_igemm_launch(const CUtensorMap *wmap, const e2e::IgemmArgs *args, unsigned tiles, void *stream);
+extern "C" int e2e_tc_conv3x3_split_launch(const float *in, long long P, int C, void *planes, void *stream);
diff --git a/e2e-asr-pytorch_b200/csrc/conv_igemm_host.cu b/e2e-asr-pytorch_b200/csrc/conv_igemm_host.cu
--- a/e2e-asr-pytorch_b200/csrc/conv_igemm_host.cu
+++ b/e2e-asr-pytorch_b200/csrc/conv_igemm_host.cu
@@ -15,6 +15,44 @@
     return (C == 128 || C == 256) && (Cout == 128 || Cout == 256);
 }
 
+bool aligned16(const void *p) { return (reinterpret_cast<uintptr_t>(p) & 15) == 0; }
+
+int check_args(const char *name, const void *in, const int *valid, int N, int H, int W, int C, const void *w, const float *bias,
+               int Cout, int epilogue, const void *out)
+{
+    if (!in || !valid || !w || !out || (epilogue != kEpiRaw && !bias)) return set_error(E2E_ERR_ARG, "%s: null pointer", name);
+    if (N <= 0 || H <= 0 || W <= 0 || epilogue < kEpiRaw || epilogue > kEpiPool)
+        return set_error(E2E_ERR_ARG, "%s: bad size or epilogue", name);
+    if (!igemm_shape_ok(C, Cout)) return set_error(E2E_ERR_UNSUPPORTED, "%s: C = %d, Cout = %d not supported", name, C, Cout);
+    if (!aligned16(in) || !aligned16(w) || !aligned16(out) || !aligned16(bias)) return set_error(E2E_ERR_ARG, "%s: misaligned buffer", name);
+    if (3 * ((long long)N * H * W + 1) > 0x7fffffffLL) return set_error(E2E_ERR_ARG, "%s: too many pixels", name);
+    return E2E_OK;
+}
+
+int launch(const char *name, const void *planes, const int *valid, int N, int H, int W, int C, const void *w, const float *bias,
+           int Cout, int epilogue, int out_planes, void *out, void *stream)
+{
+    const long long P = (long long)N * H * W;
+    const long long rows_out = epilogue == kEpiPool ? (long long)N * ((H + 1) / 2) * ((W + 1) / 2) : P;
+    const long long tiles = epilogue == kEpiPool ? (rows_out + kIgemmBM / 4 - 1) / (kIgemmBM / 4) : (rows_out + kIgemmBM - 1) / kIgemmBM;
+    EncodeTiledFn enc = tensor_map_encoder();
+    if (!enc) return set_error(E2E_ERR_LAUNCH, "%s: cuTensorMapEncodeTiled is not available from this driver", name);
+    const cuuint32_t estr[2] = {1u, 1u};
+    CUtensorMap wmap;
+    const cuuint64_t wdims[2] = {(cuuint64_t)9 * C, (cuuint64_t)3 * Cout};
+    const cuuint64_t wstrides[1] = {(cuuint64_t)9 * C * 2};
+    const cuuint32_t wbox[2] = {(cuuint32_t)kIgemmBK, (cuuint32_t)kIgemmBN};
+    const CUresult cr = enc(&wmap, CU_TENSOR_MAP_DATA_TYPE_BFLOAT16, 2, const_cast<void *>(w), wdims, wstrides, wbox, estr, CU_TENSOR_MAP_INTERLEAVE_NONE,
+             CU_TENSOR_MAP_SWIZZLE_128B, CU_TENSOR_MAP_L2_PROMOTION_L2_256B, CU_TENSOR_MAP_FLOAT_OOB_FILL_NONE);
+    if (cr != CUDA_SUCCESS) return set_error(E2E_ERR_LAUNCH, "%s: cuTensorMapEncodeTiled (weights) failed (CUresult %d)", name, (int)cr);
+
+    const IgemmArgs a = {planes, valid, bias, out, rows_out, N, H, W, C, Cout, epilogue, out_planes};
+    const int e = e2e_tc_conv3x3_igemm_launch(&wmap, &a, (unsigned)tiles, stream);
+    count_launch();
+    if (e != (int)cudaSuccess) return set_error(E2E_ERR_LAUNCH, "%s: %s", name, cudaGetErrorString((cudaError_t)e));
+    return check_launch(name);
+}
+
 }
 }
 
@@ -25,37 +63,42 @@
     return igemm_shape_ok(C, Cout) ? 1 : 0;
 }
 
+extern "C" int e2e_conv3x3_split_planes(const float *in_nhwc, int N, int H, int W, int C, void *planes, void *stream)
+{
+    const char *name = "e2e_conv3x3_split_planes";
+    if (!in_nhwc || !planes) return set_error(E2E_ERR_ARG, "%s: null pointer", name);
+    if (N <= 0 || H <= 0 || W <= 0 || C <= 0 || C % 8) return set_error(E2E_ERR_ARG, "%s: bad size", name);
+    if (!aligned16(in_nhwc) || !aligned16(planes)) return set_error(E2E_ERR_ARG, "%s: misaligned buffer", name);
+    const int e = e2e_tc_conv3x3_split_launch(in_nhwc, (long long)N * H * W, C, planes, stream);
+    count_launch();
+    if (e != (int)cudaSuccess) return set_error(E2E_ERR_LAUNCH, "%s: %s", name, cudaGetErrorString((cudaError_t)e));
+    return check_launch(name);
+}
+
+extern "C" int e2e_conv3x3_igemm_planes(const void *planes, const int *valid_rows, int N, int H, int W, int C,
+                                        const void *w_split_bf16, const float *bias, int Cout, int epilogue, int out_planes,
+                                        void *out, void *stream)
+{
+    const char *name = "e2e_conv3x3_igemm_planes";
+    const int rc = check_args(name, planes, valid_rows, N, H, W, C, w_split_bf16, bias, Cout, epilogue, out);
+    if (rc != E2E_OK) return rc;
+    if (out_planes != 0 && out_planes != 1) return set_error(E2E_ERR_ARG, "%s: out_planes must be 0 or 1", name);
+    return launch(name, planes, valid_rows, N, H, W, C, w_split_bf16, bias, Cout, epilogue, out_planes, out, stream);
+}
+
 extern "C" int e2e_conv3x3_igemm(const float *in_nhwc, const int *valid_rows, int N, int H, int W, int C,
                                  const void *w_split_bf16, const float *bias, int Cout, int epilogue, float *out, void *stream)
 {
     const char *name = "e2e_conv3x3_igemm";
-    if (!in_nhwc || !valid_rows || !w_split_bf16 || !out || (epilogue != kEpiRaw && !bias))
-        return set_error(E2E_ERR_ARG, "%s: null pointer", name);
-    if (N <= 0 || H <= 0 || W <= 0 || epilogue < kEpiRaw || epilogue > kEpiPool)
-        return set_error(E2E_ERR_ARG, "%s: bad size or epilogue", name);
-    if (!igemm_shape_ok(C, Cout)) return set_error(E2E_ERR_UNSUPPORTED, "%s: C = %d, Cout = %d not supported", name, C, Cout);
-    if ((reinterpret_cast<uintptr_t>(in_nhwc) & 15) || (reinterpret_cast<uintptr_t>(w_split_bf16) & 15) ||
-        (reinterpret_cast<uintptr_t>(out) & 15) || (reinterpret_cast<uintptr_t>(bias) & 15))
-        return set_error(E2E_ERR_ARG, "%s: misaligned buffer", name);
-    const long long rows_out = epilogue == kEpiPool ? (long long)N * ((H + 1) / 2) * ((W + 1) / 2) : (long long)N * H * W;
-    const long long tiles = epilogue == kEpiPool ? (rows_out + kIgemmBM / 4 - 1) / (kIgemmBM / 4) : (rows_out + kIgemmBM - 1) / kIgemmBM;
-    if (tiles > 0x7fffffffLL) return set_error(E2E_ERR_ARG, "%s: too many pixels", name);
-
-    EncodeTiledFn enc = tensor_map_encoder();
-    if (!enc) return set_error(E2E_ERR_LAUNCH, "%s: cuTensorMapEncodeTiled is not available from this driver", name);
-    CUtensorMap map;
-    const cuuint64_t dims[2] = {(cuuint64_t)9 * C, (cuuint64_t)3 * Cout};
-    const cuuint64_t strides[1] = {(cuuint64_t)9 * C * 2};
-    const cuuint32_t box[2] = {(cuuint32_t)kIgemmBK, (cuuint32_t)kIgemmBN};
-    const cuuint32_t estr[2] = {1u, 1u};
-    const CUresult cr = enc(&map, CU_TENSOR_MAP_DATA_TYPE_BFLOAT16, 2, const_cast<void *>(w_split_bf16), dims, strides, box, estr,
-                            CU_TENSOR_MAP_INTERLEAVE_NONE, CU_TENSOR_MAP_SWIZZLE_128B, CU_TENSOR_MAP_L2_PROMOTION_L2_256B,
-                            CU_TENSOR_MAP_FLOAT_OOB_FILL_NONE);
-    if (cr != CUDA_SUCCESS) return set_error(E2E_ERR_LAUNCH, "%s: cuTensorMapEncodeTiled failed (CUresult %d)", name, (int)cr);
-
-    const IgemmArgs a = {in_nhwc, valid_rows, bias, out, N, H, W, C, Cout, epilogue};
-    const int e = e2e_tc_conv3x3_igemm_launch(&map, &a, (unsigned)tiles, stream);
-    count_launch();
-    if (e != (int)cudaSuccess) return set_error(E2E_ERR_LAUNCH, "%s: %s", name, cudaGetErrorString((cudaError_t)e));
-    return check_launch(name);
+    const int rc = check_args(name, in_nhwc, valid_rows, N, H, W, C, w_split_bf16, bias, Cout, epilogue, out);
+    if (rc != E2E_OK) return rc;
+    const cudaStream_t s = static_cast<cudaStream_t>(stream);
+    void *planes = nullptr;
+    cudaError_t e = cudaMallocAsync(&planes, (size_t)3 * ((size_t)N * H * W + 1) * C * 2, s);
+    if (e != cudaSuccess) return set_error(E2E_ERR_LAUNCH, "%s: planes workspace: %s", name, cudaGetErrorString(e));
+    int r = e2e_conv3x3_split_planes(in_nhwc, N, H, W, C, planes, stream);
+    if (r == E2E_OK) r = launch(name, planes, valid_rows, N, H, W, C, w_split_bf16, bias, Cout, epilogue, 0, out, stream);
+    e = cudaFreeAsync(planes, s);
+    if (r == E2E_OK && e != cudaSuccess) return set_error(E2E_ERR_LAUNCH, "%s: planes workspace: %s", name, cudaGetErrorString(e));
+    return r;
 }
diff --git a/e2e-asr-pytorch_b200/model.py b/e2e-asr-pytorch_b200/model.py
--- a/e2e-asr-pytorch_b200/model.py
+++ b/e2e-asr-pytorch_b200/model.py
@@ -99,7 +99,6 @@
 
     conv_split_format = "bf16x3"
     conv_path = "igemm"
-    IGEMM_MAX_COUT = 128
 
     def _split_weights(self, conv):
         from .stepper import SplitLinear, SplitLinearF16
@@ -122,9 +121,6 @@
         from . import ops
         n, h, w, c = x.shape
         bias = conv.bias.detach().float().contiguous()
-        if (amax_in is None and self.conv_path == "igemm" and conv.out_channels <= self.IGEMM_MAX_COUT
-                and ops.conv3x3_igemm_supported(c, conv.out_channels)):
-            return ops.conv3x3_igemm(x, valid, self._igemm_weights(conv), bias, "pool" if pool else "relu")
         k = 9 * c
         lin = self._split_weights(conv)
         total = n * h * w
@@ -166,9 +162,23 @@
         amax = torch.zeros(4, dtype=torch.int32, device=feat.device) if f16 else None
         word = lambda i: amax[i:i + 1] if f16 else None
         y = ops.conv1_direct(feat, w1, convs[0].bias.detach().float().contiguous(), v1, self.freq_dim, amax_out=word(0))
-        y = self._conv_split(y, v1, convs[1], pool=True, amax_in=word(0), amax_out=word(1))
-        y = self._conv_split(y, v2, convs[2], amax_in=word(1), amax_out=word(2))
-        y = self._conv_split(y, v2, convs[3], pool=True, amax_in=word(2), amax_out=word(3))
+        if not f16 and self.conv_path == "igemm" and not getattr(self, "_wide_igemm", True):
+            y = ops.conv3x3_igemm(y, v1, self._igemm_weights(convs[1]), convs[1].bias.detach().float().contiguous(), "pool")
+            y = self._conv_split(y, v2, convs[2])
+            y = self._conv_split(y, v2, convs[3], pool=True)
+        elif not f16 and self.conv_path == "igemm" and all(ops.conv3x3_igemm_supported(c.in_channels, c.out_channels)
+                                                           for c in convs[1:]):
+            n, h, w, _ = y.shape
+            bias = lambda conv: conv.bias.detach().float().contiguous()
+            p = ops.conv3x3_igemm(y, v1, self._igemm_weights(convs[1]), bias(convs[1]), "pool", out="planes")
+            del y
+            nhw = (n, (h + 1) // 2, (w + 1) // 2)
+            p = ops.conv3x3_igemm_planes(p, v2, nhw, self._igemm_weights(convs[2]), bias(convs[2]), "relu", out="planes")
+            y = ops.conv3x3_igemm_planes(p, v2, nhw, self._igemm_weights(convs[3]), bias(convs[3]), "pool")
+        else:
+            y = self._conv_split(y, v1, convs[1], pool=True, amax_in=word(0), amax_out=word(1))
+            y = self._conv_split(y, v2, convs[2], amax_in=word(1), amax_out=word(2))
+            y = self._conv_split(y, v2, convs[3], pool=True, amax_in=word(2), amax_out=word(3))
         out = y.permute(0, 1, 3, 2).contiguous()
         return out.view(out.shape[0], out.shape[1], self.out_dim), feat_len // 4
 
diff --git a/e2e-asr-pytorch_b200/ops.py b/e2e-asr-pytorch_b200/ops.py
--- a/e2e-asr-pytorch_b200/ops.py
+++ b/e2e-asr-pytorch_b200/ops.py
@@ -398,28 +398,64 @@
 IGEMM_EPILOGUE = {"raw": 0, "relu": 1, "pool": 2}
 
 
-def conv3x3_igemm(x_nhwc, valid_rows, w_split, bias, epilogue="relu"):
-    _chk(x_nhwc, F32, "x_nhwc")
-    _chk(valid_rows, I32, "valid_rows", x_nhwc.shape[0])
+def _igemm_check(valid_rows, n, c, w_split, bias, epilogue, out):
+    _chk(valid_rows, I32, "valid_rows", n)
     _chk(w_split, torch.bfloat16, "w_split")
-    n, h, w, c = x_nhwc.shape
     if w_split.dim() != 3 or w_split.shape[0] != 3 or w_split.shape[2] != 9 * c:
         raise ValueError("w_split must be [3, Cout, 9*%d], got %s" % (c, tuple(w_split.shape)))
-    cout = w_split.shape[1]
     if epilogue not in IGEMM_EPILOGUE:
         raise ValueError("unknown epilogue " + str(epilogue))
+    if out not in ("fp32", "planes"):
+        raise ValueError("out must be 'fp32' or 'planes', got " + str(out))
+    cout = w_split.shape[1]
     if epilogue != "raw":
         _chk(bias, F32, "bias", cout)
-    if epilogue == "raw":
-        out = torch.empty((n * h * w, cout), dtype=F32, device=x_nhwc.device)
-    elif epilogue == "relu":
-        out = torch.empty((n, h, w, cout), dtype=F32, device=x_nhwc.device)
-    else:
-        out = torch.empty((n, (h + 1) // 2, (w + 1) // 2, cout), dtype=F32, device=x_nhwc.device)
+    return cout
+
+
+def _igemm_out(n, h, w, cout, epilogue, out, device):
+    shape = (n * h * w,) if epilogue == "raw" else (n, h, w) if epilogue == "relu" else (n, (h + 1) // 2, (w + 1) // 2)
+    if out == "fp32":
+        return torch.empty(shape + (cout,), dtype=F32, device=device)
+    rows = 1
+    for d in shape:
+        rows *= d
+    return torch.empty((3, rows + 1, cout), dtype=torch.bfloat16, device=device)
+
+
+def conv3x3_split_planes(x_nhwc):
+    _chk(x_nhwc, F32, "x_nhwc")
+    n, h, w, c = x_nhwc.shape
+    planes = torch.empty((3, n * h * w + 1, c), dtype=torch.bfloat16, device=x_nhwc.device)
+    L.check(L.load().e2e_conv3x3_split_planes(L.ptr(x_nhwc), n, h, w, c, L.ptr(planes), _stream()))
+    return planes
+
+
+def conv3x3_igemm(x_nhwc, valid_rows, w_split, bias, epilogue="relu", out="fp32"):
+    _chk(x_nhwc, F32, "x_nhwc")
+    n, h, w, c = x_nhwc.shape
+    cout = _igemm_check(valid_rows, n, c, w_split, bias, epilogue, out)
+    if out == "planes":
+        return conv3x3_igemm_planes(conv3x3_split_planes(x_nhwc), valid_rows, (n, h, w), w_split, bias, epilogue, out)
+    y = _igemm_out(n, h, w, cout, epilogue, out, x_nhwc.device)
     L.check(L.load().e2e_conv3x3_igemm(L.ptr(x_nhwc), L.ptr(valid_rows), n, h, w, c, L.ptr(w_split),
                                       L.ptr(bias) if epilogue != "raw" else None, int(cout), IGEMM_EPILOGUE[epilogue],
-                                      L.ptr(out), _stream()))
-    return out
+                                      L.ptr(y), _stream()))
+    return y
+
+
+def conv3x3_igemm_planes(planes, valid_rows, nhw, w_split, bias, epilogue="relu", out="fp32"):
+    _chk(planes, torch.bfloat16, "planes")
+    n, h, w = (int(d) for d in nhw)
+    if planes.dim() != 3 or planes.shape[0] != 3 or planes.shape[1] != n * h * w + 1:
+        raise ValueError("planes must be [3, %d, C], got %s" % (n * h * w + 1, tuple(planes.shape)))
+    c = planes.shape[2]
+    cout = _igemm_check(valid_rows, n, c, w_split, bias, epilogue, out)
+    y = _igemm_out(n, h, w, cout, epilogue, out, planes.device)
+    L.check(L.load().e2e_conv3x3_igemm_planes(L.ptr(planes), L.ptr(valid_rows), n, h, w, c, L.ptr(w_split),
+                                             L.ptr(bias) if epilogue != "raw" else None, int(cout), IGEMM_EPILOGUE[epilogue],
+                                             int(out == "planes"), L.ptr(y), _stream()))
+    return y
 
 
 def conv_bias_relu_mask(y_nhwc, bias, valid_rows, amax_in=None, inv_w_scale=None, amax_out=None):
diff --git a/include/e2e_asr_b200.h b/include/e2e_asr_b200.h
--- a/include/e2e_asr_b200.h
+++ b/include/e2e_asr_b200.h
@@ -130,6 +130,10 @@
                             long long first_pixel, long long n_pixels, void *stream);
 
 int e2e_conv3x3_igemm_supported(int C, int Cout);
+int e2e_conv3x3_split_planes(const float *in_nhwc, int N, int H, int W, int C, void *planes, void *stream);
+int e2e_conv3x3_igemm_planes(const void *planes, const int *valid_rows, int N, int H, int W, int C,
+                             const void *w_split_bf16, const float *bias, int Cout, int epilogue, int out_planes,
+                             void *out, void *stream);
 int e2e_conv3x3_igemm(const float *in_nhwc, const int *valid_rows, int N, int H, int W, int C,
                       const void *w_split_bf16, const float *bias, int Cout, int epilogue, float *out, void *stream);
 
```

Result: faster. 1046 (median of 6 runs) (+1.7%).
